# CERALIVE/ceracoder

Hardware: AMD Instinct MI355X
Metric: 1080p H.264 encoded frames/sec per GPU (higher is better)
Workload: dtype u8

## Files before the change

### ceracoder_amd/csrc/enc_handle.cpp

```cpp
#include "enc_internal.hpp"

std::atomic<int> g_open_encoders{0};
bool exclusive_device(const mi355enc_t *h) { static const bool env = getenv("MI355ENC_EXCLUSIVE") != nullptr; return h->cfg.exclusive_device != 0 || env; }
bool pgate_on(int nmb) {
    if (getenv("MI355ENC_NO_PGATE")) return false;
    const char *m = getenv("MI355ENC_PGATE_MAX");
    return nmb <= (m ? atoi(m) : 16384);
}
bool fip_on(int nmb) { return getenv("MI355ENC_NO_FIP") ? false : getenv("MI355ENC_FIP") ? true : nmb <= 3600; }
bool overlap_allowed(const mi355enc_t *h) {
    static const bool serial = getenv("MI355ENC_SERIAL") != nullptr;
    return !serial && h->safe_level == 0 && !h->cfg.single_stream && g_open_encoders.load(std::memory_order_relaxed) == 1;
}

int sync_compute(mi355enc_t *h) {
    if (h->ustream) HIPCHK(hipStreamSynchronize(h->ustream));
    HIPCHK(hipStreamSynchronize(h->fstream));
    HIPCHK(hipStreamSynchronize(h->stream));
    HIPCHK(hipStreamSynchronize(h->cstream));
    HIPCHK(hipStreamSynchronize(h->istream));
    return 0;
}

#include <mutex>
#include <vector>
static std::mutex g_pin_mu;
static std::vector<std::pair<uintptr_t, size_t>> g_pins;
bool host_range_pinned(const void *p, size_t bytes) {
    const uintptr_t a = (uintptr_t)p;
    std::lock_guard<std::mutex> g(g_pin_mu);
    for (const auto &r : g_pins)
        if (a >= r.first && a + bytes <= r.first + r.second) return true;
    return false;
}

extern "C" {

void *mi355enc_host_alloc(size_t bytes) {
    void *p = nullptr;
    if (!bytes || hipHostMalloc(&p, bytes, hipHostMallocPortable) != hipSuccess || !p) { (void)hipGetLastError(); return nullptr; }
    std::lock_guard<std::mutex> g(g_pin_mu);
    g_pins.emplace_back((uintptr_t)p, bytes);
    return p;
}
void mi355enc_host_free(void *p) {
    if (!p) return;
    {
        std::lock_guard<std::mutex> g(g_pin_mu);
        for (size_t i = 0; i < g_pins.size(); i++)
            if (g_pins[i].first == (uintptr_t)p) { g_pins.erase(g_pins.begin() + (long)i); break; }
    }
    (void)hipHostFree(p);
}

int mi355enc_abi_version(void) { return MI355ENC_ABI_VERSION; }

const char *mi355enc_strerror(int code) {
    switch (code) {
    case MI355ENC_OK: return "ok";
    case MI355ENC_ERR_ARG: return "invalid argument";
    case MI355ENC_ERR_NO_DEVICE: return "no usable HIP device (this encoder has no CPU fallback)";
    case MI355ENC_ERR_HIP: return "HIP runtime error";
    case MI355ENC_ERR_NOMEM: return "out of memory";
    case MI355ENC_ERR_OVERFLOW: return "output buffer too small";
    case MI355ENC_ERR_STATE: return "call order violated";
    default: return "unknown error";
    }
}

void mi355enc_default_cfg(mi355enc_cfg_t *c, int width, int height, int fps_num, int fps_den) {
    memset(c, 0, sizeof *c);
    c->width = width; c->height = height; c->fps_num = fps_num; c->fps_den = fps_den > 0 ? fps_den : 1;
    c->gop = 60; c->me_range = 16; c->bitrate_bps = 2048000; c->device_id = 0; c->fixed_qp = -1;
    c->qp_min = 10; c->qp_max = 51; c->pipeline_depth = 0; c->profile_events = 0; c->use_graphs = 1; c->keep_prefilter = 0; c->deblock_mode = 0; c->subpel = 1; c->i4x4 = 1; c->transform8x8 = 0; c->intra_in_p = 1; c->vbv_ms = 600; c->cavlc_threads = 0; c->intra_mode = 0; c->scenecut = 1; c->exclusive_device = 0; c->aq_mode = 0; c->single_stream = 0; c->intra_slices = 0; c->partitions = 0; c->profile_overlap = 0; c->i8x8 = 0; c->slices = 0; c->slice_deblock = 1;
}

int mi355enc_open(const mi355enc_cfg_t *cfg, mi355enc_t **out) {
    if (!cfg || !out) return MI355ENC_ERR_ARG;
    *out = nullptr;
    const double t_open = now_ms();
    if (cfg->width < 16 || cfg->height < 16 || cfg->width > 8192 || cfg->height > 8192 || (cfg->width & 1) || (cfg->height & 1) ||
        cfg->fps_num <= 0 || cfg->fps_den <= 0 || cfg->gop < 1 || cfg->me_range < 1 || cfg->me_range > 16 ||
        cfg->pipeline_depth < 0 || cfg->pipeline_depth > NSLOT - 1 || cfg->fixed_qp > 51 || cfg->slices < 0 || cfg->intra_slices < 0) {
        fprintf(stderr, "mi355enc: invalid configuration\n");
        return MI355ENC_ERR_ARG;
    }
    int ndev = 0;
    hipError_t e = hipGetDeviceCount(&ndev);
    if (e != hipSuccess || ndev <= 0 || cfg->device_id < 0 || cfg->device_id >= ndev) {
        fprintf(stderr, "mi355enc: no usable HIP device (count=%d, device-id=%d, %s); this encoder has no CPU path\n", ndev,
                cfg->device_id, e == hipSuccess ? "ok" : hipGetErrorString(e));
        return MI355ENC_ERR_NO_DEVICE;
    }
    HIPCHK(hipSetDevice(cfg->device_id));
    mi355enc_t *h = new (std::nothrow) mi355enc();
    if (!h) return MI355ENC_ERR_NOMEM;
    memset((void *)&h->cfg, 0, sizeof h->cfg);
    h->cfg = *cfg;
    if (h->cfg.qp_min <= 0 && h->cfg.qp_max <= 0) { h->cfg.qp_min = 10; h->cfg.qp_max = 51; }
    if (h->cfg.qp_max > 51) h->cfg.qp_max = 51;
    if (h->cfg.qp_min < 0) h->cfg.qp_min = 0;
    h->mbw = (cfg->width + 15) / 16; h->mbh = (cfg->height + 15) / 16;
    {
        const bool local = h->cfg.slice_deblock != 0;
        auto rows_for = [&](int n) { if (n <= 1) return 0; int rows = (h->mbh + n - 1) / n; if (local) rows = (rows + MI355_BAND_ROWS - 1) / MI355_BAND_ROWS * MI355_BAND_ROWS; return rows >= h->mbh ? 0 : rows; };
        static_assert(MI355_BAND_ROWS == 4, "the oracle rounds slice heights to multiples of four rows (orc_slice_rows_for)");
        const int nauto = h->mbh / 17 < 1 ? 1 : h->mbh / 17 > 8 ? 8 : h->mbh / 17;
        const int ns = h->cfg.intra_slices > 0 ? h->cfg.intra_slices : nauto, np = h->cfg.slices > 0 ? h->cfg.slices : nauto;
        h->islice_rows = rows_for(ns > h->mbh ? h->mbh : ns);
        h->pslice_rows = rows_for(np > h->mbh ? h->mbh : np);
        h->slice_dbf = local ? 2 : 0;
        h->stage_slice_rows = 0; h->stage_slice_dbf = 0;
    }
    h->W = h->mbw * 16; h->H = h->mbh * 16; h->nmb = h->mbw * h->mbh;
    h->ysz = (size_t)h->W * h->H; h->csz = h->ysz / 2;
    h->head = h->tail = h->pending = 0;
    h->cur = 0; h->have_ref = 0; h->frames_since_idr = 0; h->idr_count = 0; h->last_collected_rec = 0; h->last_slot = nullptr;
    h->ir_on = 0; h->ir_pos = 0; h->ir_R = 0; h->ir_skip_owed = 0;
    h->in_w = cfg->width; h->in_h = cfg->height; h->sar_w = h->sar_h = 0; h->scaling = false; h->d_scale_tab = nullptr; h->scale_tab_bytes = 0; memset(&h->scale, 0, sizeof h->scale);
    h->col_full = 0; h->col_prim = h->col_trc = h->col_mat = 2; h->in_col_set = false; csc_resolve(h);
    h->ov_len = 0; h->ov_last_have = 0; h->ov_last_len = 0; mi355enc_overlay_default_style(&h->ov_style);
    for (int l = 0; l < MI355ENC_IMAGE_LAYERS; l++) { h->img_cur[l] = nullptr; h->img_x[l] = h->img_y[l] = 0; h->img_op[l] = 256; h->img_serial[l] = 0; }
    h->img_bufs = nullptr; h->img_dev_bytes = 0; memset(h->img_last, 0, sizeof h->img_last);
    snapshot_init(h);
    h->q_on = false; h->q_have = false; h->d_qacc = nullptr; h->h_qres = nullptr; for (int i = 0; i < NSLOT; i++) h->ev_q[i] = nullptr; memset(&h->q_last, 0, sizeof h->q_last); memset(&h->q_tot, 0, sizeof h->q_tot);
    for (int i = 0; i < NSET; i++) { h->g_intra[i] = h->g_deblock[i] = nullptr; h->d_ctx2[i] = nullptr; h->d_surf[i] = nullptr; h->d_idec2[i] = nullptr; h->d_mbi_set[i] = nullptr; h->d_levels_set[i] = nullptr; h->d_qp_off[i] = nullptr; }
    h->prev_slot = nullptr;
    h->d_ctx = nullptr; h->d_pre_y = h->d_pre_uv = nullptr; memset(h->d_imv, 0, sizeof h->d_imv); h->d_psrc[0] = h->d_psrc[1] = nullptr; h->psrc_cur = 0; h->fstream = nullptr; h->ustream = nullptr; h->d_ip_strips = nullptr; h->epoch = 0; h->istream = nullptr; h->ev_pmb = nullptr; h->d_db_gran = nullptr; h->d_db_par = nullptr; h->d_ib_gran = nullptr; h->ev_dbI[0] = h->ev_dbI[1] = nullptr; h->dbI_busy[0] = h->dbI_busy[1] = 0; h->d_off = nullptr; h->d_isad = nullptr; h->d_dbrec = nullptr; h->d_idec = nullptr;
    h->cstream = nullptr; h->d_mbi = nullptr; h->d_levels = nullptr;
    memset(&h->st, 0, sizeof h->st);
    h->want_bps.store(cfg->bitrate_bps ? cfg->bitrate_bps : 2048000);
    h->fixed_qp.store(cfg->fixed_qp);
    h->fixed_drop.store(0);
    *out = h;
    g_open_encoders.fetch_add(1, std::memory_order_relaxed);
    HIPCHK(hipStreamCreateWithFlags(&h->stream, hipStreamNonBlocking));
    h->fip_rows = fip_on(h->nmb);
    h->pgate = pgate_on(h->nmb);
    {
        const int wgs_max = 256 - 256 / 4;
        for (int idr = 0; idr < 2; idr++) h->wait_room[idr] = wait_room_wgs(h->mbw, h->mbh, idr != 0, h->fip_rows) <= wgs_max;
    }
    for (int i = 0; i < NSET; i++) HIPCHK(hipMalloc((void **)&h->d_ctx2[i], sizeof(frame_ctx_t)));
    h->d_ctx = h->d_ctx2[0];
    if (h->cfg.single_stream) {
        h->cstream = h->fstream = h->istream = h->stream;
        HIPCHK(hipEventCreateWithFlags(&h->ev_pmb, hipEventDisableTiming));
    } else {
        int lo = 0, hi = 0;
        HIPCHK(hipDeviceGetStreamPriorityRange(&lo, &hi));
        HIPCHK(hipStreamCreateWithPriority(&h->cstream, hipStreamNonBlocking, hi));
        const char *rs = getenv("MI355ENC_RESERVE_CUS");
        const int nres = rs ? atoi(rs) : 0, rmode = (rs && strchr(rs, ',')) ? atoi(strchr(rs, ',') + 1) : 0;
        if (nres > 0 && nres < 200) {
            hipDeviceProp_t pr;
            HIPCHK(hipGetDeviceProperties(&pr, h->cfg.device_id));
            const int ncu = pr.multiProcessorCount;
            uint32_t mask[16];
            memset(mask, 0, sizeof mask);
            for (int i = 0; i < ncu && i < 512; i++) mask[i >> 5] |= 1u << (i & 31);
            for (int k = 0; k < nres; k++) { const int i = rmode == 1 ? (int)((long long)k * ncu / nres) : k; mask[i >> 5] &= ~(1u << (i & 31)); }
            HIPCHK(hipExtStreamCreateWithCUMask(&h->fstream, (uint32_t)((ncu + 31) / 32), mask));
            HIPCHK(hipExtStreamCreateWithCUMask(&h->istream, (uint32_t)((ncu + 31) / 32), mask));
        } else {
        HIPCHK(hipStreamCreateWithPriority(&h->fstream, hipStreamNonBlocking, getenv("MI355ENC_FPRIO") ? atoi(getenv("MI355ENC_FPRIO")) : lo));
        HIPCHK(hipStreamCreateWithPriority(&h->istream, hipStreamNonBlocking, 0));
        }
        if (h->cfg.pipeline_depth >= 1 && !getenv("MI355ENC_NO_UPSTREAM")) HIPCHK(hipStreamCreateWithFlags(&h->ustream, hipStreamNonBlocking));
        HIPCHK(hipEventCreateWithFlags(&h->ev_pmb, hipEventDisableTiming));
    }
    for (int i = 0; i < NSET; i++) {
        HIPCHK(hipMalloc((void **)&h->d_mbi_set[i], (size_t)h->nmb * sizeof(mb_info_t)));
        HIPCHK(hipMalloc((void **)&h->d_levels_set[i], (size_t)h->nmb * MB_LEVELS * sizeof(int16_t)));
        HIPCHK(hipMemsetAsync(h->d_mbi_set[i], 0, (size_t)h->nmb * sizeof(mb_info_t), h->stream));
    }
    h->d_mbi = h->d_mbi_set[0]; h->d_levels = h->d_levels_set[0]; h->n_submitted = 0;
    h->sc_sum = 0; h->sc_cnt = 0; h->sc_prev_skip = 0; h->sc_force_at = ~0ull;
    for (int i = 0; i < 2; i++) {
        HIPCHK(hipMalloc((void **)&h->d_rec_y[i], h->ysz + SURF_PAD));
        HIPCHK(hipMalloc((void **)&h->d_rec_uv[i], h->csz + SURF_PAD));
        HIPCHK(hipMemsetAsync(h->d_rec_y[i], 0, h->ysz + SURF_PAD, h->stream));
        HIPCHK(hipMemsetAsync(h->d_rec_uv[i], 0, h->csz + SURF_PAD, h->stream));
    }
    HIPCHK(hipMalloc((void **)&h->d_isad, (size_t)h->nmb * ISAD_PER_MB * sizeof(uint16_t)));
    HIPCHK(hipMalloc((void **)&h->d_dbrec, (size_t)h->nmb * 64));
    HIPCHK(hipMalloc((void **)&h->d_idec, (size_t)h->nmb * IDEC_BYTES + 16));
    h->d_idec2[0] = h->d_idec;
    { int r = h->words.alloc(h->mbh, h->stream); if (r) return r; }
    HIPCHK(hipMalloc((void **)&h->d_db_par, k_deblock_partab_bytes(h->mbw, h->mbh)));
    HIPCHK(hipMalloc((void **)&h->d_ib_gran, (size_t)h->mbh * h->mbw * 8 * sizeof(uint2)));
    HIPCHK(hipMemsetAsync(h->d_ib_gran, 0, (size_t)h->mbh * h->mbw * 8 * sizeof(uint2), h->stream));
    for (int i = 0; i < 2; i++) HIPCHK(hipEventCreateWithFlags(&h->ev_dbI[i], hipEventDisableTiming));
    HIPCHK(hipMalloc((void **)&h->d_db_gran, k_deblock_gran_bytes(h->mbw, h->mbh)));
    HIPCHK(hipMemsetAsync(h->d_db_gran, 0, k_deblock_gran_bytes(h->mbw, h->mbh), h->stream));
    HIPCHK(hipMalloc((void **)&h->d_off, (size_t)h->nmb * sizeof(unsigned)));
    for (int k = 0; k < NSET; k++) {
        HIPCHK(hipMalloc((void **)&h->d_surf[k], (size_t)h->nmb * SURF_U16 * sizeof(uint16_t)));
        for (int i = 0; i < 3; i++) HIPCHK(hipMalloc((void **)&h->d_imv[k][i], (size_t)h->nmb * sizeof(imv_t)));
        if (k > 0) HIPCHK(hipMalloc((void **)&h->d_idec2[k], (size_t)h->nmb * IDEC_BYTES + 16));
        if (h->cfg.aq_mode) HIPCHK(hipMalloc((void **)&h->d_qp_off[k], (size_t)h->nmb + 16));
    }
    for (int k = 0; k < 2; k++) {
        HIPCHK(hipMalloc((void **)&h->d_psrc[k], h->ysz + SURF_PAD));
        HIPCHK(hipMemsetAsync(h->d_psrc[k], 0, h->ysz + SURF_PAD, h->stream));
    }
    HIPCHK(hipMalloc((void **)&h->d_ip_strips, (size_t)h->nmb * IP_STRIP_BYTES));
    HIPCHK(hipMemsetAsync(h->d_ip_strips, 0, (size_t)h->nmb * IP_STRIP_BYTES, h->stream));
    if (cfg->keep_prefilter) {
        HIPCHK(hipMalloc((void **)&h->d_pre_y, h->ysz));
        HIPCHK(hipMalloc((void **)&h->d_pre_uv, h->csz));
    }
    for (int i = 0; i < NSLOT; i++) {
        slot_t *s = &h->slot[i];
        memset(s, 0, sizeof *s);
        HIPCHK(hipHostMalloc((void **)&s->h_ctx, sizeof(frame_ctx_t), hipHostMallocDefault));
        HIPCHK(hipHostMalloc((void **)&s->h_mbi, (size_t)h->nmb * sizeof(mb_info_t), hipHostMallocDefault));
        HIPCHK(hipHostMalloc((void **)&s->h_levels, (size_t)h->nmb * PACK_BLOCKS_MAX * 32, hipHostMallocDefault));
        HIPCHK(hipHostMalloc((void **)&s->h_hdr, (size_t)(4 + h->mbh) * sizeof(unsigned), hipHostMallocDefault));
        s->h_hdr[0] = s->h_hdr[1] = 0;
        HIPCHK(hipMalloc((void **)&s->d_src_y, h->ysz + SURF_PAD));
        HIPCHK(hipMalloc((void **)&s->d_src_uv, h->csz + SURF_PAD));
        HIPCHK(hipEventCreateWithFlags(&s->done, hipEventDisableTiming));
        HIPCHK(hipEventCreateWithFlags(&s->gpu_done, hipEventDisableTiming));
        HIPCHK(hipEventCreateWithFlags(&s->ev_front, hipEventDisableTiming));
        HIPCHK(hipEventCreateWithFlags(&s->ev_up, hipEventDisableTiming));
        for (int k = 0; k < 12; k++) HIPCHK(hipEventCreate(&s->ev[k]));
    }
    h->writer = h264_writer_new(h->mbw, h->mbh, h->cfg.transform8x8);
    if (!h->writer) return MI355ENC_ERR_NOMEM;
    h264_writer_set_slice_rows(h->writer, h->islice_rows);
    h264_writer_set_p_slices(h->writer, h->pslice_rows, h->slice_dbf);
    if (h->cfg.cavlc_threads <= 0) {
        const unsigned hw = std::thread::hardware_concurrency();
        int n = (int)(hw / 4);
        h->cfg.cavlc_threads = h->nmb < 1000 ? 1 : n < 1 ? 1 : n > 8 ? 8 : n;
    }
    if (h->cfg.cavlc_threads > 1 && h264_writer_set_threads(h->writer, h->cfg.cavlc_threads)) return MI355ENC_ERR_NOMEM;
    rc_init(&h->rc, (double)cfg->fps_num / cfg->fps_den, cfg->gop, h->want_bps.load(), h->cfg.qp_min, h->cfg.qp_max);
    if (h->cfg.vbv_ms > 0) rc_set_vbv(&h->rc, h->cfg.vbv_ms);
    HIPCHK(hipStreamSynchronize(h->stream));
    h->ms_open = now_ms() - t_open; h->n_skip_pictures = 0;
    h->safe_level = 0; h->n_recoveries = 0; h->last_error_word = 0;
    h->wk_qh = h->wk_qt = 0; h->wk_stop = false; h->wk_on = false; h->au_cap = 0;
    if (h->cfg.pipeline_depth >= 1 && !getenv("MI355ENC_SYNC_ENTROPY")) {
        h->au_cap = h264_max_au_bytes(h->mbw, h->mbh);
        for (int i = 0; i < NSLOT; i++) { h->slot[i].au = (uint8_t *)malloc(h->au_cap); if (!h->slot[i].au) return MI355ENC_ERR_NOMEM; }
        h->wk_on = true;
        h->wk = std::thread(entropy_worker, h);
    }
    h->stg_n = h->stg_next = h->stg_done = h->stg_err = 0; h->stg_gen = 0; h->stg_stop = false; h->stg_on = false;
    if (h->cfg.pipeline_depth >= 1 && !getenv("MI355ENC_NO_STAGE_THREADS")) {
        h->stg_on = true;
        for (auto &t : h->stg_th) t = std::thread(stage_helper, h);
    }
    return MI355ENC_OK;
}

void mi355enc_close(mi355enc_t *h) {
    if (!h) return;
    if (h->wk_on) {
        { std::lock_guard<std::mutex> g(h->wk_mu); h->wk_stop = true; }
        h->wk_cv.notify_all();
        h->wk.join();
        h->wk_on = false;
    }
    if (h->stg_on) {
        { std::lock_guard<std::mutex> g(h->stg_mu); h->stg_stop = true; }
        h->stg_cv.notify_all();
        for (auto &t : h->stg_th) t.join();
        h->stg_on = false;
    }
    g_open_encoders.fetch_sub(1, std::memory_order_relaxed);
    (void)hipSetDevice(h->cfg.device_id);
    if (h->ustream) { (void)hipStreamSynchronize(h->ustream); (void)hipStreamDestroy(h->ustream); }
    if (h->fstream) (void)hipStreamSynchronize(h->fstream);
    if (h->stream) (void)hipStreamSynchronize(h->stream);
    if (h->istream) (void)hipStreamSynchronize(h->istream);
    if (h->ev_pmb) (void)hipEventDestroy(h->ev_pmb);
    for (int i = 0; i < NSET; i++) { if (h->g_intra[i]) (void)hipGraphExecDestroy(h->g_intra[i]); if (h->g_deblock[i]) (void)hipGraphExecDestroy(h->g_deblock[i]); }
    for (int i = 0; i < NSLOT; i++) {
        slot_t *s = &h->slot[i];
        if (s->h_ctx) (void)hipHostFree(s->h_ctx);
        if (s->h_mbi) (void)hipHostFree(s->h_mbi);
        if (s->h_levels) (void)hipHostFree(s->h_levels);
        if (s->h_hdr) (void)hipHostFree(s->h_hdr);
        if (s->h_src) (void)hipHostFree(s->h_src);
        free(s->au);
        if (s->d_src_y) (void)hipFree(s->d_src_y);
        if (s->d_src_uv) (void)hipFree(s->d_src_uv);
        if (s->d_raw) (void)hipFree(s->d_raw);
        if (s->d_csc) (void)hipFree(s->d_csc);
        orient_free(s);
        jpeg_free(s);
        if (s->done) (void)hipEventDestroy(s->done);
        if (s->gpu_done) (void)hipEventDestroy(s->gpu_done);
        if (s->ev_front) (void)hipEventDestroy(s->ev_front);
        if (s->ev_up) (void)hipEventDestroy(s->ev_up);
        for (int k = 0; k < 12; k++) if (s->ev[k]) (void)hipEventDestroy(s->ev[k]);
    }
    for (int i = 0; i < 2; i++) { if (h->d_rec_y[i]) (void)hipFree(h->d_rec_y[i]); if (h->d_rec_uv[i]) (void)hipFree(h->d_rec_uv[i]); }
    if (h->d_pre_y) (void)hipFree(h->d_pre_y);
    if (h->d_pre_uv) (void)hipFree(h->d_pre_uv);
    if (h->d_isad) (void)hipFree(h->d_isad);
    if (h->d_dbrec) (void)hipFree(h->d_dbrec);
    if (h->d_idec) (void)hipFree(h->d_idec);
    h->words.release();
    if (h->d_db_gran) (void)hipFree(h->d_db_gran);
    if (h->d_db_par) (void)hipFree(h->d_db_par);
    if (h->d_ib_gran) (void)hipFree(h->d_ib_gran);
    for (int i = 0; i < 2; i++) if (h->ev_dbI[i]) (void)hipEventDestroy(h->ev_dbI[i]);
    if (h->d_off) (void)hipFree(h->d_off);
    scale_free(h);
    quality_free(h);
    snapshot_free(h);
    image_free(h);
    rate_free(h);
    hdr_free(h);
    adjust_free(h);
    autolevel_free(h);
    dspatial_free(h);
    lut3d_close(h);
    roi_free(h);
    mask_free(h);
    denoise_free(h);
    stab_free(h);
    warp_close(h);
    for (int k = 0; k < NSET; k++) {
        if (h->d_surf[k]) (void)hipFree(h->d_surf[k]);
        for (int i = 0; i < 3; i++) if (h->d_imv[k][i]) (void)hipFree(h->d_imv[k][i]);
        if (k > 0 && h->d_idec2[k]) (void)hipFree(h->d_idec2[k]);
        if (h->d_qp_off[k]) (void)hipFree(h->d_qp_off[k]);
    }
    for (int k = 0; k < 2; k++) if (h->d_psrc[k]) (void)hipFree(h->d_psrc[k]);
    if (h->d_ip_strips) (void)hipFree(h->d_ip_strips);
    for (int i = 0; i < NSET; i++) if (h->d_ctx2[i]) (void)hipFree(h->d_ctx2[i]);
    for (int i = 0; i < NSET; i++) { if (h->d_mbi_set[i]) (void)hipFree(h->d_mbi_set[i]); if (h->d_levels_set[i]) (void)hipFree(h->d_levels_set[i]); }
    if (h->cstream && h->cstream != h->stream) { (void)hipStreamSynchronize(h->cstream); (void)hipStreamDestroy(h->cstream); }
    if (h->fstream && h->fstream != h->stream) (void)hipStreamDestroy(h->fstream);
    if (h->istream && h->istream != h->stream) (void)hipStreamDestroy(h->istream);
    if (h->stream) (void)hipStreamDestroy(h->stream);
    h264_writer_free(h->writer);
    delete h;
}

int mi355enc_set_bitrate(mi355enc_t *h, uint32_t bps) {
    if (!h) return MI355ENC_ERR_ARG;
    h->want_bps.store(bps < 1000 ? 1000 : bps, std::memory_order_relaxed);
    return MI355ENC_OK;
}
uint32_t mi355enc_get_bitrate(const mi355enc_t *h) { return h ? h->want_bps.load(std::memory_order_relaxed) : 0; }
int mi355enc_set_fixed_qp(mi355enc_t *h, int qp) {
    if (!h || qp > 51) return MI355ENC_ERR_ARG;
    h->fixed_qp.store(qp < 0 ? -1 : qp, std::memory_order_relaxed);
    return MI355ENC_OK;
}
int mi355enc_set_fixed_drop(mi355enc_t *h, int drop) {
    if (!h || drop < 0 || (drop > DROP_MAX && drop != DROP_SKIP)) return MI355ENC_ERR_ARG;
    h->fixed_drop.store(drop, std::memory_order_relaxed);
    return MI355ENC_OK;
}
int mi355enc_set_intra_refresh(mi355enc_t *h, int on) {
    if (!h || h->n_submitted) return MI355ENC_ERR_ARG;
    if (on && (h->cfg.intra_in_p == 0 || h->cfg.partitions || h->cfg.gop < 2 || h->cfg.gop > MI355ENC_IR_MAX_PERIOD)) return MI355ENC_ERR_ARG;
    h->ir_on = on ? 1 : 0;
    return MI355ENC_OK;
}
int mi355enc_pending(const mi355enc_t *h) { return h ? h->pending : 0; }
size_t mi355enc_max_au_bytes(const mi355enc_t *h) { return h ? h264_max_au_bytes(h->mbw, h->mbh) : 0; }
int mi355enc_mb_width(const mi355enc_t *h) { return h ? h->mbw : 0; }
int mi355enc_mb_height(const mi355enc_t *h) { return h ? h->mbh : 0; }

int mi355enc_get_stats(mi355enc_t *h, mi355enc_stats_t *st) {
    if (!h || !st) return MI355ENC_ERR_ARG;
    *st = h->st;
    st->target_bps = h->want_bps.load();
    st->cavlc_threads = (uint32_t)h->cfg.cavlc_threads;
    st->ms_open = h->ms_open; st->skip_pictures = h->n_skip_pictures;
    st->recoveries = h->n_recoveries; st->last_error_word = h->last_error_word; st->safe_level = (uint32_t)h->safe_level;
    return MI355ENC_OK;
}
void mi355enc_reset_stats(mi355enc_t *h) { if (h) { memset(&h->st, 0, sizeof h->st); h->n_skip_pictures = 0; memset(&h->q_tot, 0, sizeof h->q_tot); } }

int mi355enc_fetch(mi355enc_t *h, int what, void *dst, size_t n) {
    if (!h || !dst) return MI355ENC_ERR_ARG;
    HIPCHK(hipSetDevice(h->cfg.device_id));
    const void *src = nullptr; size_t need = 0; bool host = false;
    switch (what) {
    case MI355ENC_FETCH_RECON_Y: src = h->d_rec_y[h->last_collected_rec]; need = h->ysz; break;
    case MI355ENC_FETCH_RECON_UV: src = h->d_rec_uv[h->last_collected_rec]; need = h->csz; break;
    case MI355ENC_FETCH_PREFILTER_Y: src = h->d_pre_y; need = h->ysz; break;
    case MI355ENC_FETCH_PREFILTER_UV: src = h->d_pre_uv; need = h->csz; break;
    case MI355ENC_FETCH_MBINFO: src = h->last_slot ? h->last_slot->h_mbi : nullptr; need = (size_t)h->nmb * sizeof(mb_info_t); host = true; break;
    case MI355ENC_FETCH_SOURCE_Y: src = h->last_slot && h->last_slot->src_y == h->last_slot->d_src_y ? h->last_slot->d_src_y : nullptr; need = h->ysz; break;
    case MI355ENC_FETCH_SOURCE_UV: src = h->last_slot && h->last_slot->src_y == h->last_slot->d_src_y ? h->last_slot->d_src_uv : nullptr; need = h->csz; break;
    case MI355ENC_FETCH_SCALE_TABLES: src = h->d_scale_tab; need = h->scale_tab_bytes; break;
    case MI355ENC_FETCH_LEVELS: src = h->last_slot ? h->d_levels_set[h->last_slot->set] : nullptr; need = (size_t)h->nmb * MB_LEVELS * 2; break;
    case 102: case 103: case 104: {
        if (!h->words.fetch_bytes(what)) return MI355ENC_ERR_STATE;
        if (n < h->words.fetch_bytes(what)) return MI355ENC_ERR_OVERFLOW;
        int r = sync_compute(h);
        return r ? r : h->words.fetch(what, dst);
    }
    case 100: src = h->d_dbrec; need = (size_t)h->nmb * 64; break;
    case 101: src = h->d_isad; need = 1024; break;
    default: return MI355ENC_ERR_ARG;
    }
    if (!src) return MI355ENC_ERR_STATE;
    if (n < need) return MI355ENC_ERR_OVERFLOW;
    if (host) { memcpy(dst, src, need); return MI355ENC_OK; }
    { int r = sync_compute(h); if (r) return r; }
    HIPCHK(hipMemcpy(dst, src, need, hipMemcpyDeviceToHost));
    return MI355ENC_OK;
}

}
```

### ceracoder_amd/csrc/k_motion.hip

```cpp
#include "kernels_common.hpp"

#ifndef ME_MBS
#define ME_MBS 4
#endif
#define ME_WQ (ME_MBS + 2)
#define ME_ROWS 50
#define ME_STRIDE 53
#define ME_K 5

DEV unsigned long long qsad(unsigned lo, unsigned hi, unsigned cur, unsigned long long acc) {
    unsigned long long src = ((unsigned long long)hi << 32) | lo;
    return __builtin_amdgcn_qsad_pk_u16_u8(src, cur, acc);
}
DEV int mv_bits(int v) {
    int a = iabs(v);
    return a == 0 ? 1 : 7 + 2 * (31 - __clz(a));
}
DEV int med3(int a, int b, int c) {
    const int lo = a < b ? a : b, hi = a < b ? b : a;
    return c < lo ? lo : (c > hi ? hi : c);
}
struct fpred_t { int px, py, sx, sy; };
DEV fpred_t field_pred(const imv_t *__restrict__ f, int mbw, int mx, int my, bool top) {
    const bool avA = mx > 0, avB = top, avC = top && mx + 1 < mbw, avD = mx > 0 && top, hasC = avC || avD;
    const int self = my * mbw + mx;
    const unsigned wa = avA ? ldg32(f + self - 1) : 0u, wb = avB ? ldg32(f + self - mbw) : 0u;
    const unsigned wc = avC ? ldg32(f + self - mbw + 1) : (avD ? ldg32(f + self - mbw - 1) : 0u);
    const int ax = (int)(int16_t)(wa & 0xFFFF), ay = (int)(int16_t)(wa >> 16), bx = (int)(int16_t)(wb & 0xFFFF), by = (int)(int16_t)(wb >> 16);
    const int cx = (int)(int16_t)(wc & 0xFFFF), cy = (int)(int16_t)(wc >> 16);
    const int n = (avA ? 1 : 0) + (avB ? 1 : 0) + (hasC ? 1 : 0);
    fpred_t r;
    if (n == 1) { r.px = avA ? ax : avB ? bx : cx; r.py = avA ? ay : avB ? by : cy; }
    else { r.px = med3(ax, bx, cx); r.py = med3(ay, by, cy); }
    const bool zero = !avA || !avB || wa == 0u || wb == 0u;
    r.sx = zero ? 0 : r.px; r.sy = zero ? 0 : r.py;
    return r;
}
template <bool ZERO = false>
DEV unsigned select_min(const unsigned long long *acc, int g, int dxg, bool active, int R, int lambda, int px, int py, int sx, int sy) {
    const unsigned INVALID = 0x40000000u;
    unsigned bo[4];
#pragma unroll
    for (int o = 0; o < 4; o++) {
        const int dx = -16 + 4 * dxg + o;
        bo[o] = (dx >= -R && dx <= R && active) ? (((unsigned)(lambda * mv_bits(dx - px)) << 12) | (unsigned)(dx + 16)) : INVALID;
    }
    const int so = sx + 16 - 4 * dxg;
    unsigned best = 0xFFFFFFFFu;
#pragma unroll
    for (int d = 0; d < ME_K; d++) {
        const int dy = -16 + ME_K * g + d;
        const unsigned pos = (unsigned)(dy + 16) << 6;
        const unsigned bd = (dy >= -R && dy <= R) ? (((unsigned)(lambda * (mv_bits(dy - py) + SEL_BONUS)) << 12) | pos) : INVALID;
        const unsigned lo = (unsigned)acc[d], hi = (unsigned)(acc[d] >> 32);
        unsigned s[4] = {(lo << 16) >> 4, (lo & 0xFFFF0000u) >> 4, (hi << 16) >> 4, (hi & 0xFFFF0000u) >> 4};
        unsigned k[4];
#pragma unroll
        for (int o = 0; o < 4; o++) {
            const bool is_skip = !ZERO && dy == sy && so == o && active;
            k[o] = is_skip ? (s[o] | pos | (unsigned)(sx + 16)) : s[o] + bd + bo[o];
        }
        unsigned ka = k[0] < k[1] ? k[0] : k[1], kb = k[2] < k[3] ? k[2] : k[3];
        ka = ka < kb ? ka : kb;
        best = best < ka ? best : ka;
    }
    if (ZERO && active && ME_K * g <= 16 && 16 < ME_K * g + ME_K && dxg == 4) {
        const unsigned long long a = acc[16 - ME_K * (16 / ME_K)];
        const unsigned k0 = (((unsigned)a << 16) >> 4) | (16u << 6) | 16u;
        best = best < k0 ? best : k0;
    }
    return wave64_umin(best);
}
DEV void store_imv(imv_t *dst, unsigned best, int lambda, int px, int py, int sx, int sy) {
    const int bx = (int)(best & 63) - 16, by = (int)((best >> 6) & 63) - 16;
    const unsigned bits = (bx == sx && by == sy) ? 0u : (unsigned)(mv_bits(bx - px) + mv_bits(by - py) + SEL_BONUS);
    const unsigned sad = (best >> 12) - (unsigned)lambda * bits;
    stg64(dst, make_uint2(((unsigned)(uint16_t)(4 * bx)) | ((unsigned)(uint16_t)(4 * by) << 16), sad | (bits << 16)));
}

__global__ __launch_bounds__(64 * ME_MBS) void me_kernel(const frame_ctx_t cv, int row0) {
    const frame_ctx_t *__restrict__ ctx = &cv;
    if (blockIdx.x == 0) tl_first(ctx, 0);
    __shared__ unsigned win[ME_ROWS * ME_STRIDE];
    const int stride = ctx->stride, mbw = ctx->mbw, mbh = ctx->mbh;
    const int W = mbw * 16, H = mbh * 16;
    const int strips = (mbw + ME_MBS - 1) / ME_MBS;
    const int tile = xcd_remap(blockIdx.x, gridDim.x);
    const int my = row0 + tile / strips, sx = tile % strips;
    const int t = threadIdx.x;
    const uint8_t *__restrict__ ref = ctx->me_ref_y;

    for (int i = t; i < 48 * ME_WQ; i += 64 * ME_MBS) {
        int row = i / ME_WQ, q = i - row * ME_WQ;
        const int gy = clip3(0, H - 1, my * 16 - 16 + row), gx = sx * (ME_MBS * 16) - 16 + 16 * q;
        uint4 v;
#ifdef ME_DBG_NOSTAGE
        v = make_uint4(i, i, i, i);
        if (gx != -12345) {}
#else
        if (gx >= 0 && gx < W) v = ldg128(ref + (size_t)gy * stride + gx);
#endif
        else { const unsigned e = ldg8(ref + (size_t)gy * stride + (gx < 0 ? 0 : W - 1)) * 0x01010101u; v = make_uint4(e, e, e, e); }
        unsigned *d = &win[row * ME_STRIDE + 4 * q];
        d[0] = v.x; d[1] = v.y; d[2] = v.z; d[3] = v.w;
    }
    if (t < ME_ROWS) win[t * ME_STRIDE + 4 * ME_WQ] = 0;
    if (t < 2 * (4 * ME_WQ + 1)) win[(48 + t / (4 * ME_WQ + 1)) * ME_STRIDE + t % (4 * ME_WQ + 1)] = 0;

    const int lane = t & 63, m = t >> 6;
    const int mx = sx * ME_MBS + m;
    const bool active = lane < 63 && mx < mbw;
    const int g = lane < 63 ? lane / 9 : 0, dxg = lane < 63 ? lane % 9 : 0;
    const int mxc = mx < mbw ? mx : mbw - 1;

    unsigned c[16][4];
    {
        const uint8_t *__restrict__ src = ctx->src_y;
        const int ss = ctx->src_stride, vh = ctx->vis_h;
        const int mu = __builtin_amdgcn_readfirstlane(mxc);
#pragma unroll
        for (int r = 0; r < 16; r++) {
            int sy = my * 16 + r;
            sy = sy < vh ? sy : vh - 1;
#ifdef ME_DBG_NOCUR
            const uint4 v = make_uint4(sy, mu, r, sy ^ mu);
#else
            const uint4 v = ldc128(src + (size_t)sy * ss + mu * 16);
#endif
            c[r][0] = __builtin_amdgcn_readfirstlane(v.x); c[r][1] = __builtin_amdgcn_readfirstlane(v.y);
            c[r][2] = __builtin_amdgcn_readfirstlane(v.z); c[r][3] = __builtin_amdgcn_readfirstlane(v.w);
        }
        if (lane < 16 && mx < mbw) {
            int sy = my * 16 + lane;
            sy = sy < vh ? sy : vh - 1;
            stg128(ctx->psrc_out + (size_t)(my * 16 + lane) * stride + mu * 16, ldg128(src + (size_t)sy * ss + mu * 16));
        }
    }
    __syncthreads();

    unsigned long long acc[ME_K];
#pragma unroll
    for (int d = 0; d < ME_K; d++) acc[d] = 0;
    const unsigned *wp = &win[(ME_K * g) * ME_STRIDE + 4 * m + dxg];
#ifdef ME_DBG_REPEAT
    for (int rep = 0; rep < ME_DBG_REPEAT; rep++) {
#endif
    unsigned w0 = wp[0], w1 = wp[1], w2 = wp[2], w3 = wp[3], w4 = wp[4];
#pragma unroll
    for (int j = 0; j < 16 + ME_K - 1; j++) {
        unsigned n0 = 0, n1 = 0, n2 = 0, n3 = 0, n4 = 0;
        if (j + 1 < 16 + ME_K - 1) {
            n0 = wp[(j + 1) * ME_STRIDE + 0]; n1 = wp[(j + 1) * ME_STRIDE + 1]; n2 = wp[(j + 1) * ME_STRIDE + 2];
            n3 = wp[(j + 1) * ME_STRIDE + 3]; n4 = wp[(j + 1) * ME_STRIDE + 4];
        }
#pragma unroll
        for (int d = 0; d < ME_K; d++) {
            const int r = j - d;
            if (r >= 0 && r < 16) {
                acc[d] = qsad(w0, w1, c[r][0], acc[d]);
                acc[d] = qsad(w1, w2, c[r][1], acc[d]);
                acc[d] = qsad(w2, w3, c[r][2], acc[d]);
                acc[d] = qsad(w3, w4, c[r][3], acc[d]);
            }
        }
        asm volatile("" : "+v"(acc[0]), "+v"(acc[1]), "+v"(acc[2]), "+v"(acc[3]), "+v"(acc[4]));
        __builtin_amdgcn_sched_barrier(0);
        w0 = n0; w1 = n1; w2 = n2; w3 = n3; w4 = n4;
    }
#ifdef ME_DBG_REPEAT
    }
#endif
#ifdef ME_DBG_NOSURF
    if (active && acc[0] == 0x123456789ull) {
#else
    if (active) {
#endif
        uint16_t *sf = ctx->surf + (size_t)(my * mbw + mx) * SURF_U16 + 4 * dxg;
#pragma unroll
        for (int d = 0; d < ME_K; d++) stg64(sf + (ME_K * g + d) * SURF_COLS, make_uint2((unsigned)acc[d], (unsigned)(acc[d] >> 32)));
    }
#ifdef ME_DBG_NOSEL
    const unsigned best = ((((unsigned)acc[0] ^ (unsigned)acc[4]) & 0x0FFFu) << 12) | 0x410u;
#else
    const unsigned best = select_min<true>(acc, g, dxg, active, ctx->me_range, ctx->lambda, 0, 0, 0, 0);
#endif
    if (lane == 0 && mx < mbw) store_imv(&ctx->imv_a[my * mbw + mx], best, ctx->lambda, 0, 0, 0, 0);
    tl_last(ctx, 1);
}

__global__ __launch_bounds__(256) void me_select_kernel(const frame_ctx_t cv, int mb0, int mb1, const imv_t *__restrict__ in, imv_t *__restrict__ out,
                                                        const imv_t *__restrict__ prev, int mode) {
    const frame_ctx_t *__restrict__ ctx = &cv;
    const int mbw = ctx->mbw;
    const int lane = threadIdx.x & 63, wave = __builtin_amdgcn_readfirstlane(threadIdx.x >> 6);
    const int mbn = mb0 + xcd_remap(blockIdx.x, gridDim.x) * 4 + wave;
    if (mbn >= mb1) return;
    const int my = mbn / mbw, mx = mbn - my * mbw;
    const fpred_t fp = field_pred(in, mbw, mx, my, row_has_top(ctx, my));
    const int px = fp.px >> 2, py = fp.py >> 2, sx = fp.sx >> 2, sy = fp.sy >> 2;
    if (mode) {
        fpred_t fq = {0, 0, 0, 0};
        if (mode == 2) fq = field_pred(prev, mbw, mx, my, row_has_top(ctx, my));
        if (px == (fq.px >> 2) && py == (fq.py >> 2) && sx == (fq.sx >> 2) && sy == (fq.sy >> 2)) {
            if (lane == 0) stg64(&out[mbn], ldg64(&in[mbn]));
            return;
        }
    }
    const bool active = lane < 63;
    const int g = active ? lane / 9 : 0, dxg = active ? lane % 9 : 0;
    unsigned long long acc[ME_K];
    const uint16_t *sf = ctx->surf + (size_t)mbn * SURF_U16 + 4 * dxg;
#pragma unroll
    for (int d = 0; d < ME_K; d++) { const uint2 v = ldg64(sf + (ME_K * g + d) * SURF_COLS); acc[d] = ((unsigned long long)v.y << 32) | v.x; }
    const unsigned best = select_min(acc, g, dxg, active, ctx->me_range, ctx->lambda, px, py, sx, sy);
    if (lane == 0) store_imv(&out[mbn], best, ctx->lambda, px, py, sx, sy);
}

#ifndef SEL_SPW
#define SEL_SPW 8
#endif
__global__ __launch_bounds__(256) void me_select_sparse_kernel(const frame_ctx_t cv, int mb0, int mb1, const imv_t *__restrict__ in, imv_t *__restrict__ out, const imv_t *__restrict__ prev) {
    const frame_ctx_t *__restrict__ ctx = &cv;
    const int mbw = ctx->mbw;
    const int lane = threadIdx.x & 63, wave = __builtin_amdgcn_readfirstlane(threadIdx.x >> 6);
    const int base = mb0 + ((int)blockIdx.x * 4 + wave) * SEL_SPW;
    if (base >= mb1) return;
    const int mine = base + (lane < SEL_SPW ? lane : 0);
    const bool have = lane < SEL_SPW && mine < mb1;
    const int mbn_l = have ? mine : base, my_l = mbn_l / mbw, mx_l = mbn_l - my_l * mbw;
    const bool top_l = row_has_top(ctx, my_l);
    const fpred_t fp = field_pred(in, mbw, mx_l, my_l, top_l), fq = field_pred(prev, mbw, mx_l, my_l, top_l);
    const int px = fp.px >> 2, py = fp.py >> 2, sx = fp.sx >> 2, sy = fp.sy >> 2;
    const bool same = px == (fq.px >> 2) && py == (fq.py >> 2) && sx == (fq.sx >> 2) && sy == (fq.sy >> 2);
    if (have && same) stg64(&out[mbn_l], ldg64(&in[mbn_l]));
    unsigned todo = (unsigned)(__ballot(have && !same) & ((1ull << SEL_SPW) - 1ull));
    const bool active = lane < 63;
    const int g = active ? lane / 9 : 0, dxg = active ? lane % 9 : 0;
    while (todo) {
        const int j = __builtin_ctz(todo);
        todo &= todo - 1;
        const int mbn = base + j;
        const int jpx = __builtin_amdgcn_readlane(px, j), jpy = __builtin_amdgcn_readlane(py, j), jsx = __builtin_amdgcn_readlane(sx, j), jsy = __builtin_amdgcn_readlane(sy, j);
        unsigned long long acc[ME_K];
        const uint16_t *sf = ctx->surf + (size_t)mbn * SURF_U16 + 4 * dxg;
#pragma unroll
        for (int d = 0; d < ME_K; d++) { const uint2 v = ldg64(sf + (ME_K * g + d) * SURF_COLS); acc[d] = ((unsigned long long)v.y << 32) | v.x; }
        const unsigned best = select_min(acc, g, dxg, active, ctx->me_range, ctx->lambda, jpx, jpy, jsx, jsy);
        if (lane == 0) store_imv(&out[mbn], best, ctx->lambda, jpx, jpy, jsx, jsy);
    }
}

#define SP_GS 24
#define SP_PS 20
struct sp_lds {
    uint8_t G[23 * SP_GS];
    int16_t H1[18 * SP_GS];
    uint8_t b[19 * SP_PS];
    uint8_t h[18 * SP_GS];
    uint8_t j[18 * SP_PS];
    uint8_t pad[16];
};
typedef short sp_s2 __attribute__((ext_vector_type(2)));
DEV sp_s2 as_s2(unsigned v) { return __builtin_bit_cast(sp_s2, v); }
DEV unsigned as_u(sp_s2 v) { return __builtin_bit_cast(unsigned, v); }
DEV sp_s2 bytes_lo(unsigned w) { return as_s2(__builtin_amdgcn_perm(0u, w, 0x0c010c00u)); }
DEV sp_s2 bytes_hi(unsigned w) { return as_s2(__builtin_amdgcn_perm(0u, w, 0x0c030c02u)); }
DEV sp_s2 clip255_s2(sp_s2 v) { return __builtin_elementwise_min(__builtin_elementwise_max(v, (sp_s2)(0)), (sp_s2)(255)); }
DEV sp_s2 pair_s2(int a, int b) { return as_s2(__builtin_amdgcn_perm((unsigned)b, (unsigned)a, 0x05040100u)); }
DEV unsigned pack_s2(sp_s2 lo, sp_s2 hi) { return __builtin_amdgcn_perm(as_u(hi), as_u(lo), 0x06040200u); }
DEV unsigned clip_pack4(int a, int b, int c, int d) { return pack_s2(clip255_s2(pair_s2(a, b)), clip255_s2(pair_s2(c, d))); }
DEV int mvq_bits(int q) {
    unsigned k = q > 0 ? (unsigned)(2 * q - 1) : (unsigned)(-2 * q);
    return 2 * (31 - __clz((int)(k + 1))) + 1;
}
DEV unsigned lds4(const uint8_t *plane, int o) {
    const unsigned *w = (const unsigned *)(plane + (o & ~3));
    return __builtin_amdgcn_alignbyte(w[1], w[0], (unsigned)(o & 3));
}
DEV unsigned sp_sample4(const sp_lds *L, int X, int Y, int fx, int fy) {
#define SG(x, y) lds4(L->G, ((y) + 2) * SP_GS + (x) + 2)
#define SB(x, y) lds4(L->b, (y) * SP_PS + (x))
#define SH(x, y) lds4(L->h, (y) * SP_GS + (x) + 2)
#define SJ(x, y) lds4(L->j, (y) * SP_PS + (x))
    if (fy == 0) {
        if (fx == 0) return SG(X, Y);
        return fx == 2 ? SB(X, Y) : fx == 1 ? avg4(SG(X, Y), SB(X, Y)) : avg4(SG(X + 1, Y), SB(X, Y));
    }
    if (fx == 0) return fy == 2 ? SH(X, Y) : fy == 1 ? avg4(SG(X, Y), SH(X, Y)) : avg4(SG(X, Y + 1), SH(X, Y));
    if ((fx & 1) && (fy & 1)) return avg4(fy == 1 ? SB(X, Y) : SB(X, Y + 1), fx == 1 ? SH(X, Y) : SH(X + 1, Y));
    if (fx == 2 && fy == 2) return SJ(X, Y);
    if (fx == 2) return avg4(fy == 1 ? SB(X, Y) : SB(X, Y + 1), SJ(X, Y));
    return avg4(fx == 1 ? SH(X, Y) : SH(X + 1, Y), SJ(X, Y));
#undef SG
#undef SB
#undef SH
#undef SJ
}
DEV void sp_planes(sp_lds *L, const int lane) {
    if (lane < 54) {
        const int d = lane % 6, seg = lane / 6;
        sp_s2 lo[7], hi[7];
#pragma unroll
        for (int r = 0; r < 7; r++) {
            const unsigned w = *(const unsigned *)&L->G[(2 * seg + r) * SP_GS + 4 * d];
            lo[r] = bytes_lo(w); hi[r] = bytes_hi(w);
        }
#pragma unroll
        for (int t = 0; t < 2; t++) {
            const sp_s2 vl = (lo[t + 2] + lo[t + 3]) * (sp_s2)(20) - (lo[t + 1] + lo[t + 4]) * (sp_s2)(5) + (lo[t] + lo[t + 5]);
            const sp_s2 vh = (hi[t + 2] + hi[t + 3]) * (sp_s2)(20) - (hi[t + 1] + hi[t + 4]) * (sp_s2)(5) + (hi[t] + hi[t + 5]);
            const int R = 2 * seg + t;
            unsigned *o = (unsigned *)&L->H1[R * SP_GS + 4 * d];
            o[0] = as_u(vl); o[1] = as_u(vh);
            *(unsigned *)&L->h[R * SP_GS + 4 * d] = pack_s2(clip255_s2((vl + (sp_s2)(16)) >> (sp_s2)(5)), clip255_s2((vh + (sp_s2)(16)) >> (sp_s2)(5)));
        }
    }
#pragma unroll
    for (int it = 0; it < 2; it++) {
        const int i = lane + 64 * it;
        if (i < 19 * 5) {
            const int R = i / 5, g = i - R * 5;
            const unsigned *gw = (const unsigned *)&L->G[(R + 2) * SP_GS + 4 * g];
            const unsigned d0 = gw[0] ^ 0x80808080u, d1 = gw[1] ^ 0x80808080u, d2 = gw[2] ^ 0x80808080u;
            int o[4];
#pragma unroll
            for (int k = 0; k < 4; k++) {
                const unsigned w0 = k ? __builtin_amdgcn_alignbyte(d1, d0, (unsigned)k) : d0, w1 = k ? __builtin_amdgcn_alignbyte(d2, d1, (unsigned)k) : d1;
                const int v = __builtin_amdgcn_sdot4((int)w0, 0x1414FB01, __builtin_amdgcn_sdot4((int)w1, 0x000001FB, 4096, false), false);
                o[k] = (v + 16) >> 5;
            }
            *(unsigned *)&L->b[R * SP_PS + 4 * g] = clip_pack4(o[0], o[1], o[2], o[3]);
        }
    }
    WAVE_SYNC();
#pragma unroll
    for (int it = 0; it < 2; it++) {
        const int i = lane + 64 * it;
        if (i < 18 * 5) {
            const int R = i / 5, g = i - R * 5;
            const unsigned *hw = (const unsigned *)&L->H1[R * SP_GS + 4 * g];
            const unsigned p0 = hw[0], p1 = hw[1], p2 = hw[2], p3 = hw[3], p4 = hw[4];
            const unsigned q0 = __builtin_amdgcn_alignbyte(p1, p0, 2u), q1 = __builtin_amdgcn_alignbyte(p2, p1, 2u),
                           q2 = __builtin_amdgcn_alignbyte(p3, p2, 2u), q3 = __builtin_amdgcn_alignbyte(p4, p3, 2u);
            const sp_s2 ca = {1, -5}, cb = {20, 20}, cc = {-5, 1};
#define J3(a, b, c) __builtin_amdgcn_sdot2(as_s2(a), ca, __builtin_amdgcn_sdot2(as_s2(b), cb, __builtin_amdgcn_sdot2(as_s2(c), cc, 512, false), false), false)
            const int v0 = J3(p0, p1, p2), v1 = J3(q0, q1, q2), v2 = J3(p1, p2, p3), v3 = J3(q1, q2, q3);
#undef J3
            *(unsigned *)&L->j[R * SP_PS + 4 * g] = clip_pack4(v0 >> 10, v1 >> 10, v2 >> 10, v3 >> 10);
        }
    }
    WAVE_SYNC();
}
__global__ __launch_bounds__(256) void subpel_kernel(const frame_ctx_t cv, int mb0, int mb1) {
    const frame_ctx_t *__restrict__ ctx = &cv;
    __shared__ __attribute__((aligned(16))) sp_lds LD[4];
    const int mbw = ctx->mbw, mbh = ctx->mbh, stride = ctx->stride, W = mbw * 16, H = mbh * 16;
    const int lane = threadIdx.x & 63, wave = __builtin_amdgcn_readfirstlane(threadIdx.x >> 6);
    int mbn = mb0 + blockIdx.x * 4 + wave;
    const bool ok = mbn < mb1;
    if (!ok) mbn = mb1 - 1;
    const int my = mbn / mbw, mx = mbn - my * mbw, x0 = mx * 16, y0 = my * 16;
    sp_lds *L = &LD[wave];
    const mb_info_t info = ld_mbinfo(&ctx->mbi[mbn]);
    const int ix = x0 + (info.mvx >> 2), iy = y0 + (info.mvy >> 2);
    const uint8_t *__restrict__ ref = ctx->ref_y;
    if (ix - 3 >= 0 && iy - 3 >= 0 && ((ix - 3) & ~3) + 28 <= W && iy + 19 < H) {
        const int a = (ix - 3) & 3;
        const uint8_t *base = ref + (size_t)(iy - 3) * stride + ((ix - 3) & ~3);
        for (int i = lane; i < 23 * 6; i += 64) {
            const int r = i / 6, d = i - r * 6;
            const unsigned w0 = ldg32(base + (size_t)r * stride + 4 * d), w1 = ldg32(base + (size_t)r * stride + 4 * d + 4);
            *(unsigned *)&L->G[r * SP_GS + 4 * d] = __builtin_amdgcn_alignbyte(w1, w0, (unsigned)a);
        }
    } else
        for (int i = lane; i < 23 * 23; i += 64) {
            int r = i / 23, c = i - r * 23;
            int yy = clip3(0, H - 1, iy - 3 + r), xx = clip3(0, W - 1, ix - 3 + c);
            L->G[r * SP_GS + c] = (uint8_t)ldg8(ref + (size_t)yy * stride + xx);
        }
    const int pr = lane >> 2, pc = (lane & 3) * 4;
    unsigned curw;
    {
        int sy = y0 + pr;
        sy = sy < ctx->vis_h ? sy : ctx->vis_h - 1;
        curw = ldg32(ctx->src_y + (size_t)sy * ctx->src_stride + x0 + pc);
    }
    WAVE_SYNC();
    sp_planes(L, lane);
    const int lambda = ctx->lambda;
    int bqx = info.mvx, bqy = info.mvy;
    unsigned best = info.cost;
#pragma unroll 1
    for (int step = 2; step >= 1; step--) {
        const int cqx = bqx, cqy = bqy;
        unsigned acc[4] = {0, 0, 0, 0};
#pragma unroll
        for (int c8 = 0; c8 < 8; c8++) {
            const int k = c8 < 4 ? c8 : c8 + 1;
            const int qx = cqx + (k % 3 - 1) * step, qy = cqy + (k / 3 - 1) * step;
            const int ox = qx - info.mvx, oy = qy - info.mvy;
            const int X = 1 + (ox >> 2) + pc, Y = 1 + (oy >> 2) + pr;
            const unsigned sad = __builtin_amdgcn_sad_u8(curw, sp_sample4(L, X, Y, ox & 3, oy & 3), 0u);
            acc[c8 >> 1] |= sad << (16 * (c8 & 1));
        }
#pragma unroll
        for (int q = 0; q < 4; q++) {
            acc[q] = (unsigned)wave64_sum((int)acc[q]);
        }
#pragma unroll
        for (int c8 = 0; c8 < 8; c8++) {
            const int k = c8 < 4 ? c8 : c8 + 1;
            const int qx = cqx + (k % 3 - 1) * step, qy = cqy + (k / 3 - 1) * step;
            const unsigned sad = (acc[c8 >> 1] >> (16 * (c8 & 1))) & 0xFFFFu;
            const unsigned cost = sad + (unsigned)(lambda * (mvq_bits(qx) + mvq_bits(qy)));
            if (cost < best) { best = cost; bqx = qx; bqy = qy; }
        }
    }
    if (lane == 0 && ok) {
        mb_info_t *mb = &ctx->mbi[mbn];
        stg32(&mb->mvx, ((unsigned)(uint16_t)bqx) | ((unsigned)(uint16_t)bqy << 16));
        stg32(&mb->cost, best);
    }
}

DEV int dec_score(unsigned M) { return dec_score_mask(M); }
DEV int row_or4(int v) {
    v |= __builtin_amdgcn_update_dpp(0, v, 0x128, 0xF, 0xF, false);
    v |= __builtin_amdgcn_update_dpp(0, v, 0x124, 0xF, 0xF, false);
    return v;
}
DEV unsigned ref_word4(const uint8_t *__restrict__ ref, int stride, int W, int H, int x, int y, bool inside) {
    if (inside) {
        const uint8_t *b = ref + (size_t)y * stride + (x & ~3);
        return __builtin_amdgcn_alignbyte(ldg32(b + 4), ldg32(b), (unsigned)(x & 3));
    }
    const uint8_t *r = ref + (size_t)clip3(0, H - 1, y) * stride;
    return pack4((int)ldg8(r + clip3(0, W - 1, x)), (int)ldg8(r + clip3(0, W - 1, x + 1)), (int)ldg8(r + clip3(0, W - 1, x + 2)), (int)ldg8(r + clip3(0, W - 1, x + 3)));
}
DEV void chroma_pred4(const frame_ctx_t *__restrict__ ctx, int lane, int x0, int y0, int W, int H, int mvx, int mvy, int *pd) {
    const int stride = ctx->stride;
    const int py = (lane >> 2) & 3, cby = (lane >> 4) & 1, c = (lane >> 1) & 1, cbx = lane & 1;
    const int cx0 = x0 >> 1, cy0 = y0 >> 1, cw = W >> 1, ch = H >> 1;
    const int cy = cby * 4 + py, cxb = cbx * 4;
    const int xi = mvx >> 3, yi = mvy >> 3, xf = mvx & 7, yf = mvy & 7;
    const uint8_t *__restrict__ rf = ctx->ref_uv;
    int A[5], B[5];
    if (cx0 + xi >= 0 && cx0 + xi + 9 <= cw && cy0 + yi >= 0 && cy0 + yi + 9 <= ch) {
        const int o = 2 * (cx0 + cxb + xi) + c, a = o & 3;
        const uint8_t *r0 = rf + (size_t)(cy0 + cy + yi) * stride + (o & ~3), *r1 = r0 + stride;
        const unsigned a0 = ldg32(r0), a1 = ldg32(r0 + 4), a2 = ldg32(r0 + 8), b0 = ldg32(r1), b1 = ldg32(r1 + 4), b2 = ldg32(r1 + 8);
        const unsigned sa0 = __builtin_amdgcn_alignbyte(a1, a0, (unsigned)a), sa1 = __builtin_amdgcn_alignbyte(a2, a1, (unsigned)a);
        const unsigned sb0 = __builtin_amdgcn_alignbyte(b1, b0, (unsigned)a), sb1 = __builtin_amdgcn_alignbyte(b2, b1, (unsigned)a);
        A[0] = byte_of(sa0, 0); A[1] = byte_of(sa0, 2); A[2] = byte_of(sa1, 0); A[3] = byte_of(sa1, 2); A[4] = (int)((a2 >> (8 * a)) & 255);
        B[0] = byte_of(sb0, 0); B[1] = byte_of(sb0, 2); B[2] = byte_of(sb1, 0); B[3] = byte_of(sb1, 2); B[4] = (int)((b2 >> (8 * a)) & 255);
    } else {
        const int ya = clip3(0, ch - 1, cy0 + cy + yi), yb = clip3(0, ch - 1, cy0 + cy + yi + 1);
#pragma unroll
        for (int i = 0; i < 5; i++) {
            const int xx = clip3(0, cw - 1, cx0 + cxb + i + xi);
            A[i] = (int)ldg8(rf + (size_t)ya * stride + 2 * xx + c);
            B[i] = (int)ldg8(rf + (size_t)yb * stride + 2 * xx + c);
        }
    }
    const int w00 = (8 - xf) * (8 - yf), w10 = xf * (8 - yf), w01 = (8 - xf) * yf, w11 = xf * yf;
#pragma unroll
    for (int i = 0; i < 4; i++) pd[i] = (w00 * A[i] + w10 * A[i + 1] + w01 * B[i] + w11 * B[i + 1] + 32) >> 6;
}
DEV unsigned pmb_luma_tq(const dev_tables *T, int lane, unsigned curw, unsigned pw, int qp, bool decimate, int *lev, int *x) {
    const int py = (lane >> 2) & 3, fy = ((py & 1) << 1) | (py >> 1);
    const col_bf cb = make_col_bf(py);
    const int kz0 = (int)((0xFEA9DB83C7426510ull >> (16 * fy)) & 0xFFFF);
    const qparams q = make_q(T, qp, false);
    const int mfe = py < 2 ? q.mf[0] : q.mf[2], mfo = py < 2 ? q.mf[2] : q.mf[1], ve = py < 2 ? q.v[0] : q.v[2], vo = py < 2 ? q.v[2] : q.v[1];
#pragma unroll
    for (int i = 0; i < 4; i++) x[i] = byte_of(curw, i) - byte_of(pw, i);
    fwd_rows4(x);
    unsigned m = 0, big = 0;
#pragma unroll
    for (int i = 0; i < 4; i++) {
        const int cf = fwd_col(x[i], cb);
        lev[i] = quant1(cf, (i & 1) ? mfo : mfe, q.f, q.qbits);
        m |= (lev[i] != 0 ? 1u : 0u) << ((kz0 >> (4 * i)) & 15);
        big |= (lev[i] > 1 || lev[i] < -1) ? 1u : 0u;
    }
    if (decimate) {
        const unsigned mm = (unsigned)row_or4((int)(m | (big << 16)));
        int s = (mm >> 16) ? 9 : dec_score(((mm & 0xFFFFu) << 1) | 1u);
        int s8 = s + quad_xor<1>(s);
        s8 += __shfl_xor(s8, 16, 64);
        int tot = s8 + quad_xor<2>(s8);
        tot += __shfl_xor(tot, 32, 64);
        if (s8 < 4 || tot < 6) { lev[0] = lev[1] = lev[2] = lev[3] = 0; }
    }
#pragma unroll
    for (int i = 0; i < 4; i++) x[i] = (lev[i] * ((i & 1) ? vo : ve)) << q.shift;
    const unsigned long long bal = __ballot((lev[0] | lev[1] | lev[2] | lev[3]) != 0);
    const unsigned long long t = bal | (bal >> 4) | (bal >> 8) | (bal >> 12);
    const int rb = lane & 15, rbx = blkx(rb) >> 2, rby = blky(rb) >> 2;
    return (unsigned)(__ballot(lane < 16 && ((t >> (16 * rby + rbx)) & 1)) & 0xFFFFull);
}
DEV unsigned pmb_satd(int lane, unsigned curw, unsigned pw) {
    const int py = (lane >> 2) & 3, s1 = py < 2 ? 1 : -1, s2 = (py & 1) ? -1 : 1;
    const int d0 = byte_of(curw, 0) - byte_of(pw, 0), d1 = byte_of(curw, 1) - byte_of(pw, 1), d2 = byte_of(curw, 2) - byte_of(pw, 2), d3 = byte_of(curw, 3) - byte_of(pw, 3);
    const int a = d0 + d3, b = d1 + d2, c = d1 - d2, e = d0 - d3;
    int t[4] = {a + b, e + c, a - b, e - c};
    int acc = 0;
#pragma unroll
    for (int i = 0; i < 4; i++) {
        const int u = mad24(t[i], s1, row_xor8(t[i]));
        const int w = mad24(u, s2, row_xor4(u));
        acc += iabs(w);
    }
    return (unsigned)wave64_sum(acc);
}
DEV unsigned pmb_sa8d(int lane, unsigned curw, unsigned pw) {
    const int s0 = (lane & 1) ? -1 : 1, s1 = (lane & 4) ? -1 : 1, s2 = (lane & 8) ? -1 : 1, s3 = (lane & 16) ? -1 : 1;
    const int d0 = byte_of(curw, 0) - byte_of(pw, 0), d1 = byte_of(curw, 1) - byte_of(pw, 1), d2 = byte_of(curw, 2) - byte_of(pw, 2), d3 = byte_of(curw, 3) - byte_of(pw, 3);
    const int a = d0 + d3, b = d1 + d2, c = d1 - d2, e = d0 - d3;
    int t[4] = {a + b, e + c, a - b, e - c};
    int acc = 0;
#pragma unroll
    for (int i = 0; i < 4; i++) {
        int u = mad24(t[i], s0, quad_xor<1>(t[i]));
        u = mad24(u, s1, row_xor4(u));
        u = mad24(u, s2, row_xor8(u));
        u = mad24(u, s3, __shfl_xor(u, 16, 64));
        acc += iabs(u);
    }
    return (unsigned)wave64_sum(acc);
}
DEV bool pmb_pick_t8(int lane, unsigned curw, unsigned pw) {
    const unsigned raw4 = pmb_satd(lane, curw, pw), raw8 = pmb_sa8d(lane, curw, pw);
    return __builtin_amdgcn_readfirstlane((int)(((raw8 + 2) >> 2) < (raw4 >> 1))) != 0;
}
template <bool SC1>
DEV void pmb_store_pred_only(const frame_ctx_t *__restrict__ ctx, int16_t *lv, int lane, int x0, int y0, unsigned pw, const int *pd) {
    const int stride = ctx->stride, pr = lane >> 2, pc = (lane & 3) * 4;
    stx32<SC1>(ctx->rec_y + (size_t)(y0 + pr) * stride + x0 + pc, pw);
    const int py = (lane >> 2) & 3, cby = (lane >> 4) & 1, c = (lane >> 1) & 1, cbx = lane & 1;
    const unsigned mine = pack4(pd[0], pd[1], pd[2], pd[3]), other = (unsigned)quad_xor<2>((int)mine);
    if (lane < 32 && c == 0) {
        uint2 out;
        out.x = __builtin_amdgcn_perm(other, mine, 0x05010400u);
        out.y = __builtin_amdgcn_perm(other, mine, 0x07030602u);
        stx64<SC1>(ctx->rec_uv + (size_t)((y0 >> 1) + cby * 4 + py) * stride + 2 * ((x0 >> 1) + cbx * 4), out);
    }
    if (lane < MB_LEVELS * 2 / 16) stg128(lv + 8 * lane, make_uint4(0, 0, 0, 0));
}

template <bool SC1>
DEV unsigned pmb_luma_t8(const frame_ctx_t *__restrict__ ctx, int *tile, int lane, unsigned curw, unsigned pw, int qp, int mbn, int x0, int y0) {
    const int pr = lane >> 2, pc = (lane & 3) * 4;
    {
        int *t = tile + ((pr >> 3) * 2 + (pc >> 3)) * 64 + (pr & 7) * 8 + (pc & 7);
#pragma unroll
        for (int i = 0; i < 4; i++) t[i] = byte_of(curw, i) - byte_of(pw, i);
    }
    WAVE_SYNC();
    const bool act = lane < 16;
    const int i8 = (lane >> 2) & 3, j = lane & 3;
    int *tb = tile + i8 * 64;
    const int m6 = qp % 6, k6 = qp / 6;
    int rs[2][8], cw[2][8];
    unsigned submask = 0;
    if (act) {
#pragma unroll
        for (int r = 0; r < 2; r++) {
#pragma unroll
            for (int i = 0; i < 8; i++) rs[r][i] = tb[(2 * j + r) * 8 + i];
            fdct8_1d(rs[r]);
        }
    }
    WAVE_SYNC();
    if (act) {
#pragma unroll
        for (int r = 0; r < 2; r++)
#pragma unroll
            for (int i = 0; i < 8; i++) tb[(2 * j + r) * 8 + i] = rs[r][i];
    }
    WAVE_SYNC();
    if (act) {
#pragma unroll
        for (int c2 = 0; c2 < 2; c2++) {
#pragma unroll
            for (int r = 0; r < 8; r++) cw[c2][r] = tb[r * 8 + 2 * j + c2];
            fdct8_1d(cw[c2]);
#pragma unroll
            for (int r = 0; r < 8; r++) {
                const int xx = 2 * j + c2, cl = pos_class8(r, xx);
                const int qbits = 16 + k6, f = (1 << qbits) / 6;
                const int a = iabs(cw[c2][r]);
                int l = (int)(((long long)a * g_tab.mf8[m6][cl] + f) >> qbits);
                l = l > 2047 ? 2047 : l;
                l = cw[c2][r] < 0 ? -l : l;
                const int kk = g_tab.izz8[r * 8 + xx];
                stg16(&ctx->levels[(size_t)mbn * MB_LEVELS + L_LUMA + (4 * i8 + (kk & 3)) * 16 + (kk >> 2)], l);
                if (l) submask |= 1u << (kk & 3);
                const int ls = 16 * g_tab.v8[m6][cl];
                cw[c2][r] = qp >= 36 ? (l * ls) << (k6 - 6) : (l * ls + (1 << (5 - k6))) >> (6 - k6);
            }
        }
    }
    WAVE_SYNC();
    if (act) {
#pragma unroll
        for (int c2 = 0; c2 < 2; c2++)
#pragma unroll
            for (int r = 0; r < 8; r++) tb[r * 8 + 2 * j + c2] = cw[c2][r];
    }
    submask |= (unsigned)quad_xor<1>((int)submask);
    submask |= (unsigned)quad_xor<2>((int)submask);
    WAVE_SYNC();
    if (act) {
#pragma unroll
        for (int r = 0; r < 2; r++) {
#pragma unroll
            for (int i = 0; i < 8; i++) rs[r][i] = tb[(2 * j + r) * 8 + i];
            idct8_1d(rs[r]);
        }
    }
    WAVE_SYNC();
    if (act) {
#pragma unroll
        for (int r = 0; r < 2; r++)
#pragma unroll
            for (int i = 0; i < 8; i++) tb[(2 * j + r) * 8 + i] = rs[r][i];
    }
    WAVE_SYNC();
    if (act) {
#pragma unroll
        for (int c2 = 0; c2 < 2; c2++) {
#pragma unroll
            for (int r = 0; r < 8; r++) cw[c2][r] = tb[r * 8 + 2 * j + c2];
            idct8_1d(cw[c2]);
        }
    }
    WAVE_SYNC();
    if (act) {
#pragma unroll
        for (int c2 = 0; c2 < 2; c2++)
#pragma unroll
            for (int r = 0; r < 8; r++) tb[r * 8 + 2 * j + c2] = (cw[c2][r] + 32) >> 6;
    }
    WAVE_SYNC();
    {
        const int *t = tile + ((pr >> 3) * 2 + (pc >> 3)) * 64 + (pr & 7) * 8 + (pc & 7);
        int o[4];
#pragma unroll
        for (int i = 0; i < 4; i++) o[i] = clip255(byte_of(pw, i) + t[i]);
        stx32<SC1>(ctx->rec_y + (size_t)(y0 + pr) * ctx->stride + x0 + pc, pack4(o[0], o[1], o[2], o[3]));
    }
    return (unsigned)(__ballot(act && ((submask >> j) & 1u)) & 0xFFFFull);
}
DEV unsigned part_gsum(unsigned v) {
    v += (unsigned)quad_xor<1>((int)v);
    v += (unsigned)row_xor4((int)v);
    v += (unsigned)row_xor8((int)v);
    v += (unsigned)__shfl_xor((int)v, 16, 64);
    return v;
}
DEV unsigned part_total(unsigned g) { g += (unsigned)quad_xor<2>((int)g); return g + (unsigned)__shfl_xor((int)g, 32, 64); }
#ifdef PMB_PROF
#define PMB_NPH 11
#define PMB_MARK(k) do { const unsigned long long t1_ = __builtin_readcyclecounter(); ph_[k] = t1_ - t0_; t0_ = t1_; } while (0)
#define PMB_MARK0() unsigned long long ph_[PMB_NPH] = {0, 0, 0, 0, 0, 0, 0, 0, 0, 0, 0}; unsigned long long t0_ = __builtin_readcyclecounter()
#define PMB_FLUSH() do { if (lane == 0) for (int k_ = 0; k_ < PMB_NPH; k_++) stg32((unsigned *)ctx->dbrec + (size_t)mbn * 16 + k_, (unsigned)ph_[k_]); } while (0)
#else
#define PMB_MARK(k) ((void)0)
#define PMB_MARK0() ((void)0)
#define PMB_FLUSH() ((void)0)
#endif
struct pmb_pre_t { uint2 selfw; fpred_t fp; unsigned curw; uint2 sw; unsigned ds; uint4 dw; };
DEV pmb_pre_t pmb_preload(const frame_ctx_t *__restrict__ ctx, const int mbn, const int lane) {
    const int mbw = ctx->mbw, my = mbn / mbw, mx = mbn - my * mbw, x0 = mx * 16, y0 = my * 16;
    pmb_pre_t p;
    const imv_t *__restrict__ field = k_final_imv_dev(ctx);
    p.selfw = ldg64(field + mbn);
    {
        int sy = y0 + (lane >> 2);
        sy = sy < ctx->vis_h ? sy : ctx->vis_h - 1;
        p.curw = ldg32(ctx->src_y + (size_t)sy * ctx->src_stride + x0 + (lane & 3) * 4);
    }
    {
        const int cby = (lane >> 4) & 1, cbx = lane & 1;
        int sy = (y0 >> 1) + cby * 4 + ((lane >> 2) & 3);
        const int vh2 = ctx->vis_h >> 1;
        sy = sy < vh2 ? sy : vh2 - 1;
        p.sw = ldg64(ctx->src_uv + (size_t)sy * ctx->src_stride + 2 * ((x0 >> 1) + cbx * 4));
    }
    p.dw = ctx->intra_p ? ldg128(ctx->idec + (size_t)mbn * IDEC_BYTES + 16) : make_uint4(0, 0, 0, 0);
    p.fp = field_pred(field, mbw, mx, my, row_has_top(ctx, my));
    p.ds = (unsigned)*(const GAS uint16_t *)(ctx->surf + (size_t)mbn * SURF_U16 + ((p.fp.sy >> 2) + 16) * SURF_COLS + (p.fp.sx >> 2) + 16);
    return p;
}
DEV bool ir_ok(const frame_ctx_t *__restrict__ ctx, int mx, int mvx) {
    return mx >= ctx->ir_c0 || (16 * mx + 15 + (mvx >> 2) + ((mvx & 3) ? 3 : 0) <= ctx->ir_clean && 8 * mx + 7 + (mvx >> 3) + ((mvx & 7) ? 1 : 0) <= (ctx->ir_clean >> 1));
}
DEV int ir_max_whole(const frame_ctx_t *__restrict__ ctx, int mx) {
    const int kl = ctx->ir_clean - 16 * mx - 15, kc = 2 * ((ctx->ir_clean >> 1) - 8 * mx - 7);
    return 4 * (kl < kc ? kl : kc);
}
template <bool SC1>
DEV void pmb_store_intra(mb_info_t *mb, const uint4 dw, int qp, int lane) {
    if (lane == 0) {
        const bool i4 = ((dw.x >> 16) & 255u) != 0;
        mb_info_t m;
        m.mvx = 0; m.mvy = 0; m.mb_type = i4 ? 2 : 0; m.i16_mode = i4 ? 0 : (uint8_t)(dw.x & 255u); m.chroma_mode = (uint8_t)((dw.x >> 8) & 255u);
        m.qp = (uint8_t)qp; m.nzmask = 0; m.cost = dw.y;
        st_mbinfo_x<SC1>(mb, m);
    }
}
template <bool SC1, bool PART, int T8, bool IR>
DEV void pmb_mb(const frame_ctx_t *__restrict__ ctx, sp_lds *L, const int mbn, const int lane, const int refine, const pmb_pre_t &pre) {
    const int mbw = ctx->mbw, mbh = ctx->mbh, stride = ctx->stride, W = mbw * 16, H = mbh * 16, qp = mb_qp_dev(ctx, mbn), lambda = ctx->lambda;
    const int my = mbn / mbw, mx = mbn - my * mbw, x0 = mx * 16, y0 = my * 16;
    const dev_tables *T = &g_tab;
    PMB_MARK0();
    const uint2 selfw = pre.selfw;
    int imx = (int)(int16_t)(selfw.x & 0xFFFF);
    const int imy = (int)(int16_t)(selfw.x >> 16);
    const unsigned di = selfw.y & 0xFFFFu, ibits = selfw.y >> 16;
    const fpred_t fp = pre.fp;
    const int pr = lane >> 2, pc = (lane & 3) * 4;
    const int py = (lane >> 2) & 3;
    const unsigned curw = pre.curw;
    int sv[4];
    {
        const int c = (lane >> 1) & 1;
        const uint2 sw = pre.sw;
        const unsigned slo = c ? (sw.x >> 8) : sw.x, shi = c ? (sw.y >> 8) : sw.y;
        sv[0] = (int)(slo & 255); sv[1] = (int)((slo >> 16) & 255); sv[2] = (int)(shi & 255); sv[3] = (int)((shi >> 16) & 255);
    }
    int16_t *lv = ctx->levels + (size_t)mbn * MB_LEVELS;
    mb_info_t *mb = &ctx->mbi[mbn];
    if (IR && mx >= ctx->ir_c0 && mx < ctx->ir_c1) {
        pmb_store_intra<SC1>(mb, pre.dw, qp, lane);
        PMB_FLUSH();
        return;
    }
    {
        const unsigned ds = pre.ds;
        const bool skip_ok = !IR || ir_ok(ctx, mx, fp.sx);
        bool pass = ctx->drop_sad && ds < ctx->drop_sad && skip_ok;
        const bool worth = ds <= di + (unsigned)(lambda * SKIP_MARGIN_BITS) && skip_ok;
        PMB_MARK(0);
        if (pass || worth) {
            const int X = x0 + (fp.sx >> 2), Y = y0 + (fp.sy >> 2);
            const bool inside = X >= 0 && Y >= 0 && X + 16 <= W && Y + 16 <= H;
            const unsigned pw = ref_word4(ctx->ref_y, stride, W, H, X + pc, Y + pr, inside);
            int pd[4];
            chroma_pred4(ctx, lane, x0, y0, W, H, fp.sx, fp.sy, pd);
            if (!pass) {
                int lev[4], x[4];
                if (pmb_luma_tq(T, lane, curw, pw, qp, true, lev, x) == 0) {
                    unsigned nz_c = 0, dc_c = 0;
                    chroma_rows4(ctx, T, lv, x0 >> 1, y0 >> 1, lane, pd, sv, qp, false, false, nullptr, nz_c, dc_c, true, 0, SC1);
                    pass = (nz_c | dc_c) == 0;
                }
            }
            PMB_MARK(1);
            if (pass) {
                pmb_store_pred_only<SC1>(ctx, lv, lane, x0, y0, pw, pd);
                if (lane == 0) {
                    mb_info_t m;
                    m.mvx = (int16_t)fp.sx; m.mvy = (int16_t)fp.sy; m.mb_type = 1; m.i16_mode = 0; m.chroma_mode = 0; m.qp = (uint8_t)qp; m.nzmask = 0; m.cost = di;
                    st_mbinfo_x<SC1>(mb, m);
                }
                PMB_FLUSH();
                return;
            }
        }
    }
    if (IR && !ir_ok(ctx, mx, imx)) imx = ir_max_whole(ctx, mx);
    const int ix = x0 + (imx >> 2), iy = y0 + (imy >> 2);
    const uint8_t *__restrict__ ref = ctx->ref_y;
    if (ix - 3 >= 0 && iy - 3 >= 0 && ((ix - 3) & ~3) + 28 <= W && iy + 19 < H) {
        const int a = (ix - 3) & 3;
        const uint8_t *base = ref + (size_t)(iy - 3) * stride + ((ix - 3) & ~3);
        for (int i = lane; i < 23 * 6; i += 64) {
            const int r = i / 6, d = i - r * 6;
            const unsigned w0 = ldg32(base + (size_t)r * stride + 4 * d), w1 = ldg32(base + (size_t)r * stride + 4 * d + 4);
            *(unsigned *)&L->G[r * SP_GS + 4 * d] = __builtin_amdgcn_alignbyte(w1, w0, (unsigned)a);
        }
    } else
        for (int i = lane; i < 23 * 23; i += 64) {
            int r = i / 23, c = i - r * 23;
            int yy = clip3(0, H - 1, iy - 3 + r), xx = clip3(0, W - 1, ix - 3 + c);
            L->G[r * SP_GS + c] = (uint8_t)ldg8(ref + (size_t)yy * stride + xx);
        }
    WAVE_SYNC();
    PMB_MARK(2);
    int bqx = imx, bqy = imy;
    unsigned q0 = 0, qh[4] = {0, 0, 0, 0}, qq[4] = {0, 0, 0, 0};
    int hbx = imx, hby = imy;
    unsigned best;
    if (PART) {
        q0 = part_gsum(__builtin_amdgcn_sad_u8(curw, sp_sample4(L, 1 + pc, 1 + pr, 0, 0), 0u));
        best = part_total(q0) + (unsigned)(lambda * (mvq_bits(imx - fp.px) + mvq_bits(imy - fp.py)));
    } else
        best = (unsigned)wave64_sum((int)__builtin_amdgcn_sad_u8(curw, sp_sample4(L, 1 + pc, 1 + pr, 0, 0), 0u)) +
               (unsigned)(lambda * (mvq_bits(imx - fp.px) + mvq_bits(imy - fp.py)));
    PMB_MARK(3);
    if (refine) {
        sp_planes(L, lane);
        PMB_MARK(4);
        {
            const int cqx = bqx, cqy = bqy;
            unsigned acc[4] = {0, 0, 0, 0};
#pragma unroll
            for (int c8 = 0; c8 < 8; c8++) {
                const int k = c8 < 4 ? c8 : c8 + 1;
                const int qx = cqx + (k % 3 - 1) * 2, qy = cqy + (k / 3 - 1) * 2;
                const int ox = qx - imx, oy = qy - imy;
                const unsigned sad = __builtin_amdgcn_sad_u8(curw, sp_sample4(L, 1 + (ox >> 2) + pc, 1 + (oy >> 2) + pr, ox & 3, oy & 3), 0u);
                acc[c8 >> 1] |= sad << (16 * (c8 & 1));
            }
#pragma unroll
            for (int q = 0; q < 4; q++) {
                if (PART) { qh[q] = part_gsum(acc[q]); acc[q] = part_total(qh[q]); }
                else acc[q] = (unsigned)wave64_sum((int)acc[q]);
            }
#pragma unroll
            for (int c8 = 0; c8 < 8; c8++) {
                const int k = c8 < 4 ? c8 : c8 + 1;
                const int qx = cqx + (k % 3 - 1) * 2, qy = cqy + (k / 3 - 1) * 2;
                const unsigned sad = (acc[c8 >> 1] >> (16 * (c8 & 1))) & 0xFFFFu;
                const unsigned cost = sad + (unsigned)(lambda * (mvq_bits(qx - fp.px) + mvq_bits(qy - fp.py)));
                if (cost < best && (!IR || ir_ok(ctx, mx, qx))) { best = cost; bqx = qx; bqy = qy; }
            }
        }
        hbx = bqx; hby = bqy;
        PMB_MARK(5);
        {
            const int cqx = bqx, cqy = bqy;
            {
                const int ox = cqx - imx, oy = cqy - imy;
                best = (pmb_satd(lane, curw, sp_sample4(L, 1 + (ox >> 2) + pc, 1 + (oy >> 2) + pr, ox & 3, oy & 3)) >> 1) +
                       (unsigned)(lambda * (mvq_bits(cqx - fp.px) + mvq_bits(cqy - fp.py)));
            }
#pragma unroll 1
            for (int k = 0; k < 9; k++) {
                if (k == 4) continue;
                const int qx = cqx + (k % 3 - 1), qy = cqy + (k / 3 - 1);
                const int ox = qx - imx, oy = qy - imy;
                const unsigned cw = sp_sample4(L, 1 + (ox >> 2) + pc, 1 + (oy >> 2) + pr, ox & 3, oy & 3);
                if (PART) {
                    const int c8 = k < 4 ? k : k - 1;
                    const unsigned g = part_gsum(__builtin_amdgcn_sad_u8(curw, cw, 0u)) << (16 * (c8 & 1));
                    qq[0] |= (c8 >> 1) == 0 ? g : 0u; qq[1] |= (c8 >> 1) == 1 ? g : 0u; qq[2] |= (c8 >> 1) == 2 ? g : 0u; qq[3] |= (c8 >> 1) == 3 ? g : 0u;
                }
                const unsigned d = pmb_satd(lane, curw, cw) >> 1;
                const unsigned cost = d + (unsigned)(lambda * (mvq_bits(qx - fp.px) + mvq_bits(qy - fp.py)));
                if (cost < best && (!IR || ir_ok(ctx, mx, qx))) { best = cost; bqx = qx; bqy = qy; }
            }
        }
    }
    PMB_MARK(6);
    const int ox = bqx - imx, oy = bqy - imy;
    unsigned pw = sp_sample4(L, 1 + (ox >> 2) + pc, 1 + (oy >> 2) + pr, ox & 3, oy & 3);
    unsigned dsad = (unsigned)wave64_sum((int)__builtin_amdgcn_sad_u8(curw, pw, 0u));
    unsigned jinter = dsad + (unsigned)(lambda * (mvq_bits(bqx - fp.px) + mvq_bits(bqy - fp.py)));
    int shape = 0, lvx = bqx, lvy = bqy;
    if (PART && refine) {
        unsigned k8 = 0xFFFFFFFFu, k168 = 0xFFFFFFFFu, k816 = 0xFFFFFFFFu;
#pragma unroll 1
        for (int k = 0; k < 17; k++) {
            const int cx = k == 0 ? imx : k < 9 ? imx + (((k - 1 < 4 ? k - 1 : k) % 3) - 1) * 2 : hbx + (((k - 9 < 4 ? k - 9 : k - 8) % 3) - 1);
            const int cy = k == 0 ? imy : k < 9 ? imy + (((k - 1 < 4 ? k - 1 : k) / 3) - 1) * 2 : hby + (((k - 9 < 4 ? k - 9 : k - 8) / 3) - 1);
            const unsigned bits = (unsigned)(lambda * (mvq_bits(cx - fp.px) + mvq_bits(cy - fp.py)));
            const int c8 = k == 0 ? 0 : k < 9 ? k - 1 : k - 9;
            const unsigned pk = k == 0 ? q0 : k < 9 ? ((c8 >> 1) == 0 ? qh[0] : (c8 >> 1) == 1 ? qh[1] : (c8 >> 1) == 2 ? qh[2] : qh[3])
                                                    : ((c8 >> 1) == 0 ? qq[0] : (c8 >> 1) == 1 ? qq[1] : (c8 >> 1) == 2 ? qq[2] : qq[3]);
            const unsigned sq = k == 0 ? pk : (pk >> (16 * (c8 & 1))) & 0xFFFFu;
            const unsigned sh = sq + (unsigned)quad_xor<2>((int)sq);
            const unsigned sv_ = sq + (unsigned)__shfl_xor((int)sq, 32, 64);
            const unsigned a = ((sq + bits) << 5) | (unsigned)k, b = ((sh + bits) << 5) | (unsigned)k, c = ((sv_ + bits) << 5) | (unsigned)k;
            k8 = a < k8 ? a : k8; k168 = b < k168 ? b : k168; k816 = c < k816 ? c : k816;
        }
        const unsigned c8x8 = (k8 >> 5), c168 = (k168 >> 5), c816 = (k816 >> 5);
        unsigned t8 = c8x8 + (unsigned)quad_xor<2>((int)c8x8); t8 += (unsigned)__shfl_xor((int)t8, 32, 64);
        const unsigned t168 = c168 + (unsigned)__shfl_xor((int)c168, 32, 64);
        const unsigned t816 = c816 + (unsigned)quad_xor<2>((int)c816);
        unsigned jb = jinter + (unsigned)lambda;
        unsigned key = 0;
        const unsigned j1 = t168 + 3u * (unsigned)lambda, j2 = t816 + 3u * (unsigned)lambda, j3 = t8 + 9u * (unsigned)lambda;
        if (j1 < jb) { jb = j1; shape = 1; key = k168; }
        if (j2 < jb) { jb = j2; shape = 2; key = k816; }
        if (j3 < jb) { jb = j3; shape = 3; key = k8; }
        shape = __builtin_amdgcn_readfirstlane(shape);
        if (shape) {
            const int k = (int)(key & 31u);
            lvx = k == 0 ? imx : k < 9 ? imx + (((k - 1 < 4 ? k - 1 : k) % 3) - 1) * 2 : hbx + (((k - 9 < 4 ? k - 9 : k - 8) % 3) - 1);
            lvy = k == 0 ? imy : k < 9 ? imy + (((k - 1 < 4 ? k - 1 : k) / 3) - 1) * 2 : hby + (((k - 9 < 4 ? k - 9 : k - 8) / 3) - 1);
            const int px_ = lvx - imx, py_ = lvy - imy;
            pw = sp_sample4(L, 1 + (px_ >> 2) + pc, 1 + (py_ >> 2) + pr, px_ & 3, py_ & 3);
            dsad = (unsigned)wave64_sum((int)__builtin_amdgcn_sad_u8(curw, pw, 0u));
            jinter = jb - (unsigned)lambda;
        }
    }
    if (ctx->intra_p && di + (unsigned)lambda * ibits >= INTRA_GATE(lambda)) {
        const uint4 dw = pre.dw;
        const unsigned jintra = dw.z + (dw.z >> 3) + (unsigned)(lambda * 12);
        if (jintra < jinter) {
            pmb_store_intra<SC1>(mb, dw, qp, lane);
            PMB_FLUSH();
            return;
        }
    }
    PMB_MARK(7);
    int pd[4];
    unsigned slot = 0;
    if (PART && shape) {
        const int src = (((lane >> 4) & 1) << 5) | ((lane & 1) << 1);
        const int cvx = __shfl(lvx, src, 64), cvy = __shfl(lvy, src, 64);
        chroma_pred4(ctx, lane, x0, y0, W, H, cvx, cvy, pd);
        const unsigned mine = ((unsigned)(uint16_t)lvx) | ((unsigned)(uint16_t)lvy << 16);
        const unsigned v1 = (unsigned)__shfl((int)mine, shape == 1 ? 32 : 2, 64), v2 = (unsigned)__shfl((int)mine, 32, 64), v3 = (unsigned)__shfl((int)mine, 34, 64);
        slot = lane == 0 ? v1 : (shape == 3 && lane == 1) ? v2 : (shape == 3 && lane == 2) ? v3 : 0u;
        bqx = __builtin_amdgcn_readfirstlane(lvx); bqy = __builtin_amdgcn_readfirstlane(lvy);
    } else chroma_pred4(ctx, lane, x0, y0, W, H, bqx, bqy, pd);
    if (ctx->drop_sad && dsad < ctx->drop_sad) {
        pmb_store_pred_only<SC1>(ctx, lv, lane, x0, y0, pw, pd);
        if (PART && shape && lane < 8) stx32<SC1>(lv + L_LDC + 2 * lane, slot);
        if (lane == 0) {
            mb_info_t m;
            m.mvx = (int16_t)bqx; m.mvy = (int16_t)bqy; m.mb_type = 1; m.i16_mode = (uint8_t)shape; m.chroma_mode = 0; m.qp = (uint8_t)qp; m.nzmask = 0; m.cost = di;
            st_mbinfo_x<SC1>(mb, m);
        }
        PMB_FLUSH();
        return;
    }
    PMB_MARK(8);
    unsigned nz_luma;
    const bool t8 = T8 == 1 || (T8 == 2 && pmb_pick_t8(lane, curw, pw));
    if (t8) {
        nz_luma = pmb_luma_t8<SC1>(ctx, (int *)L, lane, curw, pw, qp, mbn, x0, y0);
    } else {
        const int fy = ((py & 1) << 1) | (py >> 1);
        const col_bf cb = make_col_bf(py);
        const int kz0 = (int)((0xFEA9DB83C7426510ull >> (16 * fy)) & 0xFFFF);
        int lev[4], x[4];
        nz_luma = pmb_luma_tq(T, lane, curw, pw, qp, true, lev, x);
        const int bx = lane & 3, by = lane >> 4, b = ((by >> 1) << 3) | ((bx >> 1) << 2) | ((by & 1) << 1) | (bx & 1);
#pragma unroll
        for (int i = 0; i < 4; i++) stg16(&lv[L_LUMA + b * 16 + ((kz0 >> (4 * i)) & 15)], lev[i]);
        inv_rows4(x);
        int o[4];
#pragma unroll
        for (int i = 0; i < 4; i++) o[i] = clip255(byte_of(pw, i) + ((inv_col(x[i], cb) + 32) >> 6));
        stx32<SC1>(ctx->rec_y + (size_t)(y0 + pr) * stride + x0 + pc, pack4(o[0], o[1], o[2], o[3]));
    }
    PMB_MARK(9);
    unsigned nz_c = 0, dc_c = 0;
    chroma_rows4(ctx, T, lv, x0 >> 1, y0 >> 1, lane, pd, sv, qp, false, true, nullptr, nz_c, dc_c, true, 0, SC1);
    PMB_MARK(10);
    if (lane == 0) {
        unsigned nzm = nz_luma | (nz_c << 16);
        if (dc_c & 1) nzm |= NZ_CBDC;
        if (dc_c & 2) nzm |= NZ_CRDC;
        if (t8 && nz_luma) nzm |= NZ_T8;
        mb_info_t m;
        m.mvx = (int16_t)bqx; m.mvy = (int16_t)bqy; m.mb_type = 1; m.i16_mode = (uint8_t)shape; m.chroma_mode = 0; m.qp = (uint8_t)qp; m.nzmask = nzm; m.cost = di;
        st_mbinfo_x<SC1>(mb, m);
    }
    if (PART && shape) { if (lane < 8) stx32<SC1>(lv + L_LDC + 2 * lane, slot); }
    else if (lane < 2) stg128(lv + L_LDC + 8 * lane, make_uint4(0, 0, 0, 0));
    PMB_FLUSH();
}

template <bool GATED, bool ROWS, bool PART, int T8, bool IR = false>
__global__ __launch_bounds__(256) void pmb_kernel(const frame_ctx_t cv, int mb0, int mb1, int refine, const unsigned *__restrict__ gate_done, unsigned ref_epoch, unsigned *err, unsigned *row_done) {
    const frame_ctx_t *__restrict__ ctx = &cv;
    __shared__ __attribute__((aligned(16))) sp_lds LD[4];
    const int lane = threadIdx.x & 63, wave = __builtin_amdgcn_readfirstlane(threadIdx.x >> 6);
    const int mbn = mb0 + 4 * (int)blockIdx.x + wave;
    if (mb0 == 0 && blockIdx.x == 0) tl_first(ctx, 2);
    pmb_pre_t pre;
    if (mbn < mb1) pre = pmb_preload(ctx, mbn, lane);
    if (GATED) {
        if (wave == 0) {
            const int mbw = ctx->mbw, mbh = ctx->mbh;
            const int first = mb0 + 4 * (int)blockIdx.x, last = first + 3 < mb1 ? first + 3 : mb1 - 1;
            int r_lo = first / mbw - 2, r_hi = last / mbw + 2;
            r_lo = r_lo > 0 ? r_lo : 0;
            r_hi = r_hi < mbh ? r_hi : mbh - 1;
            const uint2 *flags = (const uint2 *)(gate_done + DB_DONE_STRIDE * (blockIdx.x & (DB_DONE_COPIES - 1)));
            const int b_hi = r_hi / MI355_BAND_ROWS;
            int spins = 0, b = r_lo / MI355_BAND_ROWS;
            for (;;) {
                const uint2 f = ld64_sc1(flags + b);
                if (f.x == ref_epoch && f.y == ref_epoch) { if (++b > b_hi) break; continue; }
#ifndef PMB_POLL_SLEEP
#define PMB_POLL_SLEEP 64
#endif
                __builtin_amdgcn_s_sleep(PMB_POLL_SLEEP);
                if (++spins > DB_SPIN_MAX) { st_sc1(err, 3u); break; }
                if ((spins & 255) == 0 && ld_sc1(err)) break;
            }
            __builtin_amdgcn_fence(__ATOMIC_ACQUIRE, "agent");
        }
        __syncthreads();
        tl_last(ctx, 3);
    }
    if (mbn >= mb1) return;
    pmb_mb<ROWS, PART, T8, IR>(ctx, &LD[wave], mbn, lane, refine, pre);
    if (ROWS) {
        asm volatile("s_waitcnt vmcnt(0)" ::: "memory");
        if (lane == 0) __hip_atomic_fetch_add(row_done + (mbn / ctx->mbw) * MI355_PROG_STRIDE, 1u, __ATOMIC_RELAXED, __HIP_MEMORY_SCOPE_AGENT);
    }
    tl_last(ctx, 4);
}

__global__ __launch_bounds__(256) void copy_luma_kernel(const frame_ctx_t cv) {
    const frame_ctx_t *__restrict__ ctx = &cv;
    const int W = ctx->mbw * 16, H = ctx->mbh * 16, per_row = W / 16;
    const int i = blockIdx.x * 256 + threadIdx.x;
    if (i >= per_row * H) return;
    const int y = i / per_row, x = (i - y * per_row) * 16;
    const int sy = y < ctx->vis_h ? y : ctx->vis_h - 1;
    stg128(ctx->psrc_out + (size_t)y * ctx->stride + x, ldg128(ctx->src_y + (size_t)sy * ctx->src_stride + x));
}
void k_launch_copy_luma(const frame_ctx_t *h_ctx, hipStream_t s) {
    const int n = h_ctx->mbw * h_ctx->mbh * 16;
    hipLaunchKernelGGL(copy_luma_kernel, dim3((n + 255) / 256), dim3(256), 0, s, *h_ctx);
}

__global__ __launch_bounds__(256) void imv_to_mbi_kernel(const frame_ctx_t cv, int mb0, int mb1) {
    const frame_ctx_t *__restrict__ ctx = &cv;
    const int i = mb0 + blockIdx.x * 256 + threadIdx.x;
    if (i >= mb1) return;
    const uint2 w = ldg64(k_final_imv_dev(ctx) + i);
    const int vx = (int)(int16_t)(w.x & 0xFFFF), vy = (int)(int16_t)(w.x >> 16);
    stg32(&ctx->mbi[i].mvx, w.x);
    stg32(&ctx->mbi[i].cost, (w.y & 0xFFFFu) + (unsigned)(ctx->lambda * (mvq_bits(vx) + mvq_bits(vy))));
}

void k_launch_me(const frame_ctx_t *h_ctx, int mbw, hipStream_t s) {
    int strips = (mbw + ME_MBS - 1) / ME_MBS;
    if (h_ctx->mbh > 0) hipLaunchKernelGGL(me_kernel, dim3(strips * h_ctx->mbh), dim3(64 * ME_MBS), 0, s, *h_ctx, 0);
}
void k_launch_me_select(const frame_ctx_t *h_ctx, int mbw, const imv_t *in, imv_t *out, const imv_t *prev, int mode, hipStream_t s) {
    int n = mbw * h_ctx->mbh;
    if (n <= 0) return;
    if (mode == 2) hipLaunchKernelGGL(me_select_sparse_kernel, dim3((n + 4 * SEL_SPW - 1) / (4 * SEL_SPW)), dim3(256), 0, s, *h_ctx, 0, n, in, out, prev);
    else hipLaunchKernelGGL(me_select_kernel, dim3((n + 3) / 4), dim3(256), 0, s, *h_ctx, 0, n, in, out, prev, mode);
}
void k_launch_me_select_all(const frame_ctx_t *h_ctx, int mbw, hipStream_t s) {
    imv_t *const f[3] = {h_ctx->imv_a, h_ctx->imv_b, h_ctx->imv_c};
    for (int it = 0; it < ME_ITERS; it++) k_launch_me_select(h_ctx, mbw, f[it % 3], f[(it + 1) % 3], it ? f[(it - 1) % 3] : nullptr, it ? 2 : 1, s);
}
const imv_t *k_final_imv(const frame_ctx_t *h_ctx) { return ME_ITERS % 3 == 0 ? h_ctx->imv_a : ME_ITERS % 3 == 1 ? h_ctx->imv_b : h_ctx->imv_c; }
void k_launch_subpel(const frame_ctx_t *h_ctx, int mbw, hipStream_t s) {
    const int n = mbw * h_ctx->mbh;
    if (n > 0) hipLaunchKernelGGL(subpel_kernel, dim3((n + 3) / 4), dim3(256), 0, s, *h_ctx, 0, n);
}
typedef void (*pmb_fn_t)(const frame_ctx_t, int, int, int, const unsigned *, unsigned, unsigned *, unsigned *);
#define PMB_GATES(P, T, IR) {pmb_kernel<false, false, P, T, IR>, pmb_kernel<true, false, P, T, IR>, pmb_kernel<true, true, P, T, IR>}
static const pmb_fn_t k_pmb_table[2][4][3] = {
    {PMB_GATES(false, 0, false), PMB_GATES(true, 0, false), PMB_GATES(false, 1, false), PMB_GATES(false, 2, false)},
    {PMB_GATES(false, 0, true), {nullptr, nullptr, nullptr}, PMB_GATES(false, 1, true), PMB_GATES(false, 2, true)}};
#undef PMB_GATES
int k_launch_pmb(const frame_ctx_t *h_ctx, int mbw, const pmb_launch_t *l, hipStream_t s) {
    const int n = mbw * h_ctx->mbh;
    if (n <= 0) return 0;
    if ((l->gate != PMB_IN_ORDER && !l->gate_done) || (l->gate == PMB_GATED_ROWS && !l->row_done) || l->gate < PMB_IN_ORDER || l->gate > PMB_GATED_ROWS) return -1;
    const int ir = h_ctx->ir_c1 > 0;
    const int body = h_ctx->t8 == 2 ? 3 : h_ctx->t8 ? 2 : (!ir && h_ctx->partitions) ? 1 : 0;
    hipLaunchKernelGGL(k_pmb_table[ir][body][l->gate], dim3((n + 3) / 4), dim3(256), 0, s, *h_ctx, 0, n, l->refine, l->gate_done, l->ref_epoch, l->err, l->row_done);
    return 0;
}
```

### ceracoder_amd/csrc/mi355enc_dev.h

```cpp
#ifndef MI355ENC_DEV_H
#define MI355ENC_DEV_H
#include <stdint.h>

#ifdef __cplusplus
extern "C" {
#endif

typedef struct {
    int16_t mvx, mvy;
    uint8_t mb_type;
    uint8_t i16_mode;
    uint8_t chroma_mode;
    uint8_t qp;
    uint32_t nzmask;
    uint32_t cost;
} mb_info_t;

typedef struct {
    int16_t mvx, mvy;
    uint16_t sad;
    uint16_t bits;
} imv_t;

#define MB_LEVELS 408
#define ISAD_PER_MB 152
#define IDEC_BYTES 32
#define SURF_COLS 36
#define SURF_ROWS 35
#define SURF_U16 (SURF_ROWS * SURF_COLS)
#ifndef MI355_BAND_ROWS
#define MI355_BAND_ROWS 4
#endif
#ifndef DB_CUT_MIN_MBW
#define DB_CUT_MIN_MBW 60
#endif
#ifndef MI355_PROG_STRIDE
#define MI355_PROG_STRIDE 1024
#endif
#define IP_STRIP_BYTES 64
#define ME_ITERS 3
#define SEL_BONUS 2
#define SKIP_MARGIN_BITS 4
#define INTRA_GATE(lambda) (768u + 8u * (unsigned)(lambda))
#define DROP_MAX 12
#define DROP_SKIP 255
#define L_LUMA 0
#define L_LDC 256
#define L_CDC 272
#define L_CAC 280
#define NZ_LDC (1u << 24)
#define NZ_CBDC (1u << 25)
#define NZ_CRDC (1u << 26)
#define NZ_T8 (1u << 27)
#define PACK_BLOCKS_MAX 27

typedef struct {
    const uint8_t *src_y, *src_uv;
    const uint8_t *ref_y, *ref_uv;
    uint8_t *rec_y, *rec_uv;
    mb_info_t *mbi;
    int16_t *levels;
    uint16_t *isad;
    uint8_t *idec;
    uint8_t *dbrec;
    int32_t src_stride;
    int32_t stride;
    int32_t mbw, mbh, vis_h;
    int32_t qp, me_range, lambda;
    int32_t i4x4;
    int32_t t8;
    int32_t all_intra;
    const uint8_t *me_ref_y;
    uint8_t *psrc_out;
    uint16_t *surf;
    imv_t *imv_a, *imv_b, *imv_c;
    uint32_t epoch;
    uint32_t drop_sad;
    int32_t iac_drop;
    int32_t intra_p;
    const int8_t *qp_off;
    int32_t partitions;
    int32_t slice_rows;
    int32_t slice_dbf;
    int32_t i8;
    int32_t ir_c0, ir_c1;
    int32_t ir_clean;
} frame_ctx_t;

typedef enum { DB_ALL_INTRA, DB_P, DB_P_FOLLOWS_IP, DB_P_FUSED_IP } db_variant_t;
typedef enum { PMB_IN_ORDER, PMB_GATED, PMB_GATED_ROWS } pmb_gate_t;
typedef struct { int counted, grid; } db_wgs_t;
static inline db_wgs_t db_launch_wgs(int mbh, db_variant_t v, int parts, int qpc) {
    db_wgs_t w;
    w.counted = (parts ? 4 : 2) * ((mbh + MI355_BAND_ROWS - 1) / MI355_BAND_ROWS);
    w.grid = w.counted + (v == DB_P_FUSED_IP ? mbh : qpc ? 1 : 0);
    return w;
}
typedef struct {
    db_variant_t variant;
    int parts;
    int qpc;
    int ib_rows;
    unsigned *err;
    void *gran;
    unsigned *partab;
    unsigned *band_done;
    unsigned *started;
    const unsigned *iband_done;
    const unsigned *row_done;
    unsigned row_need;
    unsigned *ip_progress;
    uint8_t *ip_strips;
    unsigned *ip_done;
    unsigned *qpc_word; unsigned qpc_base;
    unsigned *part_cnt;
} db_launch_t;
typedef struct {
    pmb_gate_t gate;
    int refine;
    const unsigned *gate_done; unsigned ref_epoch;
    unsigned *row_done;
    unsigned *err;
} pmb_launch_t;

#ifdef __cplusplus
}
#endif

#ifdef __HIPCC__
#include <hip/hip_runtime.h>
#include "mask_host.h"
void k_launch_me(const frame_ctx_t *h_ctx, int mbw, hipStream_t s);
void k_launch_copy_luma(const frame_ctx_t *h_ctx, hipStream_t s);
void k_launch_me_select(const frame_ctx_t *h_ctx, int mbw, const imv_t *in, imv_t *out, const imv_t *prev, int mode, hipStream_t s);
void k_launch_me_select_all(const frame_ctx_t *h_ctx, int mbw, hipStream_t s);
void k_launch_intra_p(const frame_ctx_t *h_ctx, int mbw, int mbh, unsigned *d_progress , uint8_t *d_strips ,
                      unsigned *d_err, hipStream_t s);
const imv_t *k_final_imv(const frame_ctx_t *h_ctx);
void k_launch_subpel(const frame_ctx_t *h_ctx, int mbw, hipStream_t s);
int k_launch_pmb(const frame_ctx_t *h_ctx, int mbw, const pmb_launch_t *l, hipStream_t s);
void k_launch_inter(const frame_ctx_t *h_ctx, int mbw, hipStream_t s);
void k_launch_intra_analyse(const frame_ctx_t *h_ctx, int mbw, int mbh, int gate_p, hipStream_t s);
void k_launch_intra_diag(const frame_ctx_t *d_ctx, int mbw, int mbh, int diag, hipStream_t s);
void k_launch_deblock_diag(const frame_ctx_t *d_ctx, int mbw, int mbh, int diag, hipStream_t s);
int k_deblock_bands16(int mbh);
int k_launch_deblock_bands(const frame_ctx_t *h_ctx, const db_launch_t *l, hipStream_t s);
size_t k_deblock_part_bytes(int mbh);
int k_intra_band_rows(void);
size_t k_deblock_partab_bytes(int mbw, int mbh);
size_t k_deblock_gran_bytes(int mbw, int mbh);
void k_launch_wait_started(const unsigned *d_started, unsigned count, unsigned *d_err, hipStream_t s);
size_t k_deblock_done_bytes(void);
void k_launch_pad(uint8_t *y, uint8_t *uv, int stride, int vis_w, int vis_h, int W, int H, hipStream_t s);
int k_intra_diags(int mbw, int mbh);
int k_intra_bands(int mbh);
void k_launch_intra_band(const frame_ctx_t *h_ctx, int mbh, uint2 *d_gran, unsigned *d_err, unsigned *d_band_done, hipStream_t s);
void k_launch_intra_rows(const frame_ctx_t *h_ctx, int mbh, uint2 *d_gran, unsigned *d_err, unsigned *d_row_done, hipStream_t s);
int k_launch_csc(int fmt, const uint8_t *p0, const uint8_t *p1, const uint8_t *p2, int s0, int s1, int s2, uint8_t *dy, uint8_t *duv,
                 int vw, int vh, int W, int H, hipStream_t s);
int k_launch_csc2(int fmt, const uint8_t *p0, const uint8_t *p1, const uint8_t *p2, int s0, int s1, int s2, uint8_t *dy, uint8_t *duv,
                  int vw, int vh, int W, int H, const int *coef, hipStream_t s);
int k_launch_hdr(int fmt, int hlg, const uint8_t *const planes[3], const int strides[3], uint8_t *dy, uint8_t *duv, int vw, int vh, int W, int H, const int *d_tables, hipStream_t s);
int k_launch_yuv_convert(uint8_t *y, uint8_t *uv, int W, int H, const int rect[4], const int *coef, hipStream_t s);
int k_launch_adjust(uint8_t *y, uint8_t *uv, int W, int H, const int rect[4], const uint8_t *luma, const int *chroma, hipStream_t s);
int k_launch_adjust_sharpen(const uint8_t *y, uint8_t *out, int W, int H, int vw, int vh, const int rect[4], const uint8_t *luma, int amount, int thr, hipStream_t s);
int k_launch_denoise(uint8_t *y, uint8_t *uv, uint16_t *hy, uint16_t *huv, int W, int H, int vw, int vh, int lmode, int cmode, const uint8_t *tabs, hipStream_t s);
int k_launch_denoise_search(const uint8_t *y, const uint16_t *hy, unsigned *vec, int W, int H, int vw, int vh, int range, int lambda, hipStream_t s);
int k_launch_denoise_mc(uint8_t *y, uint8_t *uv, const uint16_t *hy, const uint16_t *huv, uint16_t *ny, uint16_t *nuv, const unsigned *vec, int W, int H, int vw, int vh,
                        int lmode, int cmode, const uint8_t *tabs, hipStream_t s);
#define SCALE_TABLES 5
#define SCALE_TILE_W 64
#define SCALE_TILE_H 16
#define SCALE_CHUNK 8
typedef struct {
    int in_w, in_h, out_w, out_h;
    const int *first[SCALE_TABLES];
    const int16_t *q[SCALE_TABLES];
    int taps[SCALE_TABLES];
    int hrows[3];
    int span[2];
    int geom, plain;
    int lo[SCALE_TABLES], hi[SCALE_TABLES];
    int dx, dy, dw, dh;
    int border[3];
    int cap_taps[SCALE_TABLES];
} scale_plan_t;
int k_launch_scale(int fmt, const uint8_t *p0, const uint8_t *p1, const uint8_t *p2, int s0, int s1, int s2, uint8_t *dy, uint8_t *duv,
                   int W, int H, const scale_plan_t *plan, hipStream_t s, const int *stab = nullptr);
int k_launch_warp(const uint8_t *sy, const uint8_t *suv, uint8_t *dy, uint8_t *duv, int w, int h, int W, int H, const int32_t *mesh, int kind, const uint8_t fill[3], hipStream_t s, int staging = 1);
int k_launch_stab_project(const uint8_t *luma, int stride, int step, int w, int h, unsigned *sums, hipStream_t s);
int k_launch_stab_match(const unsigned *prev, const unsigned *cur, int w, int h, int range, int leak, int prime, const int bounds[4], int *state, int *rec, hipStream_t s);
int k_launch_autolevel_measure(const uint8_t *y, const uint8_t *uv, int W, int H, const int rect[4], int vw, int vh, int full_range, int reach, unsigned *slabs, hipStream_t s);
int k_launch_autolevel_decide(const unsigned *slabs, int nslabs, unsigned NC, const int set[7], int full_range, int prime, int *state, int *rec, hipStream_t s);
int k_launch_autolevel_apply(uint8_t *y, uint8_t *uv, int W, int H, const int rect[4], int luma, int chroma, const int *rec, hipStream_t s);
int k_launch_dspatial_filter(const uint8_t *src, uint8_t *out, int W, int H, int vw, int vh, const int rect[4], int chroma, const uint8_t *weight, const int *rec, const uint8_t *tabs, hipStream_t s);
int k_launch_dspatial_measure(const uint8_t *y, int W, int H, const int rect[4], int vw, int vh, int full_range, unsigned *slabs, hipStream_t s);
int k_launch_dspatial_decide(const unsigned *slabs, int nslabs, unsigned NC, const int set[5], int prime, int *state, int *rec, hipStream_t s);
int k_launch_lut3d(uint8_t *y, uint8_t *uv, int W, int H, int vw, int vh, const int rect[4], const uint32_t *nodes, int N, int strength, const int32_t coef[19], int form, hipStream_t s);
void k_launch_pack(const mb_info_t *d_mbi, const int16_t *d_levels, int nmb, int mbw, unsigned *d_off, mb_info_t *h_mbi, int16_t *h_packed,
                   unsigned *h_hdr, const unsigned *d_err, hipStream_t s);
int k_deblock_diags(int mbw, int mbh);
void k_launch_aq(const frame_ctx_t *h_ctx, int8_t *d_off, hipStream_t s);
void k_launch_qp_chain(mb_info_t *d_mbi, int nmb, int slice_qp, int slice_mbs, hipStream_t s);
void k_launch_roi_compose(const int8_t *t, int8_t *d_off, int nmb, int have_aq, hipStream_t s);
int k_launch_mask(uint8_t *y, uint8_t *uv, int W, int H, int vw, int vh, const mask_tab_t *tab, uint8_t *res, uint8_t *pa, uint8_t *pb, size_t plane_bytes, int parts, int *launches, hipStream_t s);
#define QUALITY_WORDS 8
#define QUALITY_SHARDS 32
#define QUALITY_SHARD_STRIDE 512
#define QUALITY_TICKET_WORD 8
#define QUALITY_ACC_WORDS (QUALITY_SHARDS * QUALITY_SHARD_STRIDE)
typedef struct {
    uint8_t *y, *uv;
    int32_t stride, vw, vh, W, H;
    int32_t bx, by, bw, bh;
    int32_t gx0, gy0, gx1, gy1;
    int32_t scale, halign, shaded, nlines, maxlen;
    uint8_t text[256];
    uint8_t line_end[256];
} overlay_args_t;
void k_launch_overlay(const overlay_args_t *a, hipStream_t s);
typedef struct {
    uint8_t *y, *uv;
    const uint32_t *img;
    int32_t stride, vw, vh, W, H;
    int32_t iw, ih, x, y0, opacity;
    int32_t gx0, gy0, gx1, gy1;
} image_args_t;
int k_launch_image_prepare(uint32_t *pix, size_t n, int fmt, const int *coef, hipStream_t s);
bool k_image_grid(image_args_t *a);
void k_launch_image_blend(const image_args_t *a, hipStream_t s);
int k_launch_jpeg(const int16_t *d_coef, const uint16_t *d_qt, int hs, int vs, int comps, int vw, int vh, uint8_t *dy, uint8_t *duv, int W, int H,
                  uint8_t *d_planar, hipStream_t s);
int k_launch_orient(int method, const uint8_t *sy, int ssy, const uint8_t *suv, int ssuv, int in_w, int in_h, uint8_t *dy, uint8_t *duv, int W, int H, hipStream_t s);
int k_launch_snapshot(const uint8_t *sy, int ys, const uint8_t *suv, int uvs, int w, int h, int log2s, const void *d_tab, int16_t *levels, uint8_t *hint, hipStream_t s);
int k_launch_rate_mix(const uint8_t *a_y, const uint8_t *a_uv, const uint8_t *b_y, const uint8_t *b_uv, uint8_t *o_y, uint8_t *o_uv, uint8_t *k_y, uint8_t *k_uv,
                      int W, int H, int w256, hipStream_t s);
void k_launch_quality(const uint8_t *src_y, const uint8_t *src_uv, int src_stride, const uint8_t *rec_y, const uint8_t *rec_uv, int rec_stride,
                      int width, int height, unsigned long long *d_acc, unsigned long long *out, hipStream_t s);
#endif
#endif
```

Baseline: 7470.

## Prefetch subpel window and chroma neighborhood into LDS, batch qpel SATD reductions

Splits the reference-window and chroma loads in the P macroblock kernel into issue and consume phases so they can be issued early (optionally before integer search, controlled by a new pmb_early ctx field) and land in LDS. Chroma prediction now reads from an LDS neighborhood instead of global memory. In the non-partition path, the nine quarter-pel candidates are sampled with a table-driven operand fetch and their Hadamard sums are reduced together with batched DPP steps instead of nine separate wave reductions. It also adds LDS use per block and caps SGPRs, which may affect occupancy and register pressure.

Result: no change. 7548, median of 2 (+1.0%).

```diff
diff --git a/ceracoder_amd/csrc/enc_handle.cpp b/ceracoder_amd/csrc/enc_handle.cpp
--- a/ceracoder_amd/csrc/enc_handle.cpp
+++ b/ceracoder_amd/csrc/enc_handle.cpp
@@ -214,6 +214,11 @@
         slot_t *s = &h->slot[i];
         memset(s, 0, sizeof *s);
         HIPCHK(hipHostMalloc((void **)&s->h_ctx, sizeof(frame_ctx_t), hipHostMallocDefault));
+        memset(s->h_ctx, 0, sizeof(frame_ctx_t));
+        {
+            const char *pe = getenv("MI355ENC_PMB_EARLY");
+            s->h_ctx->pmb_early = !pe ? 0 : atoi(pe) ? 1 : 2;
+        }
         HIPCHK(hipHostMalloc((void **)&s->h_mbi, (size_t)h->nmb * sizeof(mb_info_t), hipHostMallocDefault));
         HIPCHK(hipHostMalloc((void **)&s->h_levels, (size_t)h->nmb * PACK_BLOCKS_MAX * 32, hipHostMallocDefault));
         HIPCHK(hipHostMalloc((void **)&s->h_hdr, (size_t)(4 + h->mbh) * sizeof(unsigned), hipHostMallocDefault));
diff --git a/ceracoder_amd/csrc/k_motion.hip b/ceracoder_amd/csrc/k_motion.hip
--- a/ceracoder_amd/csrc/k_motion.hip
+++ b/ceracoder_amd/csrc/k_motion.hip
@@ -296,6 +296,20 @@
 #undef SH
 #undef SJ
 }
+DEV unsigned sp_operand4(const sp_lds *L, int op, int Xs, int Ys, int l24, int l20) {
+    const int P = op & 3, dx = (op >> 2) & 1, dy = (op >> 3) & 1;
+    const unsigned long long bases = (unsigned long long)offsetof(sp_lds, G) | (unsigned long long)offsetof(sp_lds, b) << 16 | (unsigned long long)offsetof(sp_lds, h) << 32 |
+                                     (unsigned long long)offsetof(sp_lds, j) << 48;
+    const int base = (int)((bases >> (16 * P)) & 0xFFFFu), stride = (P & 1) ? SP_PS : SP_GS;
+    const int s = base + (Ys + dy + (P == 0 ? 2 : 0)) * stride + Xs + dx + ((P & 1) ? 0 : 2);
+    const unsigned *w = (const unsigned *)((const uint8_t *)L + (s & ~3) + ((P & 1) ? l20 : l24));
+    return __builtin_amdgcn_alignbyte(w[1], w[0], (unsigned)(s & 3));
+}
+DEV unsigned sp_sample4_flat(const sp_lds *L, int Xs, int Ys, int l24, int l20, int fx, int fy) {
+    const int idx = fx + 4 * fy;
+    const int code = (int)(((idx < 8 ? 0x6131212014111000ull : 0x6939292836333222ull) >> (8 * (idx & 7))) & 255u);
+    return avg4(sp_operand4(L, code & 15, Xs, Ys, l24, l20), sp_operand4(L, code >> 4, Xs, Ys, l24, l20));
+}
 DEV void sp_planes(sp_lds *L, const int lane) {
     if (lane < 54) {
         const int d = lane % 6, seg = lane / 6;
@@ -429,42 +443,111 @@
     v |= __builtin_amdgcn_update_dpp(0, v, 0x124, 0xF, 0xF, false);
     return v;
 }
+DEV void ref_word4_ask_in(const uint8_t *__restrict__ ref, int stride, int x, int y, unsigned *w) {
+    const uint8_t *b = ref + (size_t)y * stride + (x & ~3);
+    w[0] = ldg32(b); w[1] = ldg32(b + 4);
+}
+DEV unsigned ref_word4_take_in(const unsigned *w, int x) { return __builtin_amdgcn_alignbyte(w[1], w[0], (unsigned)(x & 3)); }
+DEV void ref_word4_ask_cl(const uint8_t *__restrict__ ref, int stride, int W, int H, int x, int y, unsigned *b) {
+    const uint8_t *r = ref + (size_t)clip3(0, H - 1, y) * stride;
+#pragma unroll
+    for (int i = 0; i < 4; i++) b[i] = ldg8(r + clip3(0, W - 1, x + i));
+}
+DEV unsigned ref_word4_take_cl(const unsigned *b) { return pack4((int)b[0], (int)b[1], (int)b[2], (int)b[3]); }
 DEV unsigned ref_word4(const uint8_t *__restrict__ ref, int stride, int W, int H, int x, int y, bool inside) {
-    if (inside) {
-        const uint8_t *b = ref + (size_t)y * stride + (x & ~3);
-        return __builtin_amdgcn_alignbyte(ldg32(b + 4), ldg32(b), (unsigned)(x & 3));
-    }
-    const uint8_t *r = ref + (size_t)clip3(0, H - 1, y) * stride;
-    return pack4((int)ldg8(r + clip3(0, W - 1, x)), (int)ldg8(r + clip3(0, W - 1, x + 1)), (int)ldg8(r + clip3(0, W - 1, x + 2)), (int)ldg8(r + clip3(0, W - 1, x + 3)));
-}
-DEV void chroma_pred4(const frame_ctx_t *__restrict__ ctx, int lane, int x0, int y0, int W, int H, int mvx, int mvy, int *pd) {
+    unsigned w[2], b[4];
+    if (inside) { ref_word4_ask_in(ref, stride, x, y, w); return ref_word4_take_in(w, x); }
+    ref_word4_ask_cl(ref, stride, W, H, x, y, b);
+    return ref_word4_take_cl(b);
+}
+DEV int chroma_pred4_room(int x0, int y0, int W, int H, int mvx, int mvy) {
+    const int x = (x0 >> 1) + (mvx >> 3), y = (y0 >> 1) + (mvy >> 3);
+    return x | ((W >> 1) - 9 - x) | y | ((H >> 1) - 9 - y);
+}
+DEV bool chroma_pred4_inside(int x0, int y0, int W, int H, int mvx, int mvy) { return chroma_pred4_room(x0, y0, W, H, mvx, mvy) >= 0; }
+DEV void chroma_pred4_ask_in(const frame_ctx_t *__restrict__ ctx, int lane, int x0, int y0, int mvx, int mvy, unsigned *w) {
+    const int stride = ctx->stride;
+    const int py = (lane >> 2) & 3, cby = (lane >> 4) & 1, c = (lane >> 1) & 1, cbx = lane & 1;
+    const int o = 2 * ((x0 >> 1) + cbx * 4 + (mvx >> 3)) + c;
+    const uint8_t *r0 = ctx->ref_uv + (size_t)((y0 >> 1) + cby * 4 + py + (mvy >> 3)) * stride + (o & ~3), *r1 = r0 + stride;
+    w[0] = ldg32(r0); w[1] = ldg32(r0 + 4); w[2] = ldg32(r0 + 8); w[3] = ldg32(r1); w[4] = ldg32(r1 + 4); w[5] = ldg32(r1 + 8);
+}
+DEV void chroma_pred4_ask_cl(const frame_ctx_t *__restrict__ ctx, int lane, int x0, int y0, int W, int H, int mvx, int mvy, unsigned *b) {
     const int stride = ctx->stride;
     const int py = (lane >> 2) & 3, cby = (lane >> 4) & 1, c = (lane >> 1) & 1, cbx = lane & 1;
     const int cx0 = x0 >> 1, cy0 = y0 >> 1, cw = W >> 1, ch = H >> 1;
     const int cy = cby * 4 + py, cxb = cbx * 4;
-    const int xi = mvx >> 3, yi = mvy >> 3, xf = mvx & 7, yf = mvy & 7;
+    const int xi = mvx >> 3, yi = mvy >> 3;
     const uint8_t *__restrict__ rf = ctx->ref_uv;
+    const int ya = clip3(0, ch - 1, cy0 + cy + yi), yb = clip3(0, ch - 1, cy0 + cy + yi + 1);
+#pragma unroll
+    for (int i = 0; i < 5; i++) {
+        const int xx = clip3(0, cw - 1, cx0 + cxb + i + xi);
+        b[i] = ldg8(rf + (size_t)ya * stride + 2 * xx + c);
+        b[5 + i] = ldg8(rf + (size_t)yb * stride + 2 * xx + c);
+    }
+}
+DEV void chroma_bilin4(const int *A, const int *B, int mvx, int mvy, int *pd) {
+    const int xf = mvx & 7, yf = mvy & 7;
+    const int w00 = (8 - xf) * (8 - yf), w10 = xf * (8 - yf), w01 = (8 - xf) * yf, w11 = xf * yf;
+#pragma unroll
+    for (int i = 0; i < 4; i++) pd[i] = (w00 * A[i] + w10 * A[i + 1] + w01 * B[i] + w11 * B[i + 1] + 32) >> 6;
+}
+DEV void chroma_bilin4_words(unsigned a0, unsigned a1, unsigned a2, unsigned b0, unsigned b1, unsigned b2, int a, int mvx, int mvy, int *pd) {
+    const unsigned sa0 = __builtin_amdgcn_alignbyte(a1, a0, (unsigned)a), sa1 = __builtin_amdgcn_alignbyte(a2, a1, (unsigned)a);
+    const unsigned sb0 = __builtin_amdgcn_alignbyte(b1, b0, (unsigned)a), sb1 = __builtin_amdgcn_alignbyte(b2, b1, (unsigned)a);
+    const int A[5] = {byte_of(sa0, 0), byte_of(sa0, 2), byte_of(sa1, 0), byte_of(sa1, 2), (int)((a2 >> (8 * a)) & 255)};
+    const int B[5] = {byte_of(sb0, 0), byte_of(sb0, 2), byte_of(sb1, 0), byte_of(sb1, 2), (int)((b2 >> (8 * a)) & 255)};
+    chroma_bilin4(A, B, mvx, mvy, pd);
+}
+DEV void chroma_pred4_take_in(int lane, int x0, int mvx, int mvy, const unsigned *w, int *pd) {
+    const int c = (lane >> 1) & 1, cbx = lane & 1;
+    chroma_bilin4_words(w[0], w[1], w[2], w[3], w[4], w[5], (2 * ((x0 >> 1) + cbx * 4 + (mvx >> 3)) + c) & 3, mvx, mvy, pd);
+}
+DEV void chroma_pred4_take_cl(int mvx, int mvy, const unsigned *b, int *pd) {
     int A[5], B[5];
-    if (cx0 + xi >= 0 && cx0 + xi + 9 <= cw && cy0 + yi >= 0 && cy0 + yi + 9 <= ch) {
-        const int o = 2 * (cx0 + cxb + xi) + c, a = o & 3;
-        const uint8_t *r0 = rf + (size_t)(cy0 + cy + yi) * stride + (o & ~3), *r1 = r0 + stride;
-        const unsigned a0 = ldg32(r0), a1 = ldg32(r0 + 4), a2 = ldg32(r0 + 8), b0 = ldg32(r1), b1 = ldg32(r1 + 4), b2 = ldg32(r1 + 8);
-        const unsigned sa0 = __builtin_amdgcn_alignbyte(a1, a0, (unsigned)a), sa1 = __builtin_amdgcn_alignbyte(a2, a1, (unsigned)a);
-        const unsigned sb0 = __builtin_amdgcn_alignbyte(b1, b0, (unsigned)a), sb1 = __builtin_amdgcn_alignbyte(b2, b1, (unsigned)a);
-        A[0] = byte_of(sa0, 0); A[1] = byte_of(sa0, 2); A[2] = byte_of(sa1, 0); A[3] = byte_of(sa1, 2); A[4] = (int)((a2 >> (8 * a)) & 255);
-        B[0] = byte_of(sb0, 0); B[1] = byte_of(sb0, 2); B[2] = byte_of(sb1, 0); B[3] = byte_of(sb1, 2); B[4] = (int)((b2 >> (8 * a)) & 255);
-    } else {
-        const int ya = clip3(0, ch - 1, cy0 + cy + yi), yb = clip3(0, ch - 1, cy0 + cy + yi + 1);
-#pragma unroll
-        for (int i = 0; i < 5; i++) {
-            const int xx = clip3(0, cw - 1, cx0 + cxb + i + xi);
-            A[i] = (int)ldg8(rf + (size_t)ya * stride + 2 * xx + c);
-            B[i] = (int)ldg8(rf + (size_t)yb * stride + 2 * xx + c);
-        }
-    }
-    const int w00 = (8 - xf) * (8 - yf), w10 = xf * (8 - yf), w01 = (8 - xf) * yf, w11 = xf * yf;
-#pragma unroll
-    for (int i = 0; i < 4; i++) pd[i] = (w00 * A[i] + w10 * A[i + 1] + w01 * B[i] + w11 * B[i + 1] + 32) >> 6;
+#pragma unroll
+    for (int i = 0; i < 5; i++) { A[i] = (int)b[i]; B[i] = (int)b[5 + i]; }
+    chroma_bilin4(A, B, mvx, mvy, pd);
+}
+DEV void chroma_pred4(const frame_ctx_t *__restrict__ ctx, int lane, int x0, int y0, int W, int H, int mvx, int mvy, int *pd) {
+    unsigned w[6], b[10];
+    if (chroma_pred4_inside(x0, y0, W, H, mvx, mvy)) { chroma_pred4_ask_in(ctx, lane, x0, y0, mvx, mvy, w); chroma_pred4_take_in(lane, x0, mvx, mvy, w, pd); }
+    else { chroma_pred4_ask_cl(ctx, lane, x0, y0, W, H, mvx, mvy, b); chroma_pred4_take_cl(mvx, mvy, b, pd); }
+}
+#define CN_STRIDE 24
+#define CN_BYTES (10 * CN_STRIDE)
+DEV int chroma_nb_room(int nx, int ny, int W, int H) { return nx | ny | (W - CN_STRIDE - ((2 * nx) & ~3)) | ((H >> 1) - 10 - ny); }
+DEV bool chroma_nb_inside(int nx, int ny, int W, int H) { return chroma_nb_room(nx, ny, W, H) >= 0; }
+DEV unsigned chroma_nb_ask_in(const frame_ctx_t *__restrict__ ctx, int lane, int nx, int ny) {
+    const int i = lane < 60 ? lane : 59, r = i / 6, d = i - r * 6;
+    return ldg32(ctx->ref_uv + (size_t)(ny + r) * ctx->stride + ((2 * nx) & ~3) + 4 * d);
+}
+DEV void chroma_nb_take_in(uint8_t *CN, int lane, unsigned w) { if (lane < 60) *(unsigned *)&CN[4 * lane] = w; }
+DEV void chroma_nb_ask_cl(const frame_ctx_t *__restrict__ ctx, int lane, int nx, int ny, int W, int H, unsigned *b) {
+    const int cw = W >> 1, ch = H >> 1;
+#pragma unroll
+    for (int k = 0; k < 4; k++) {
+        int i = lane + 64 * k;
+        i = i < 200 ? i : 199;
+        const int r = i / 20, o = i - r * 20;
+        b[k] = ldg8(ctx->ref_uv + (size_t)clip3(0, ch - 1, ny + r) * ctx->stride + 2 * clip3(0, cw - 1, nx + (o >> 1)) + (o & 1));
+    }
+}
+DEV void chroma_nb_take_cl(uint8_t *CN, int lane, const unsigned *b) {
+#pragma unroll
+    for (int k = 0; k < 4; k++) {
+        const int i = lane + 64 * k, r = i / 20, o = i - r * 20;
+        if (i < 200) CN[r * CN_STRIDE + o] = (uint8_t)b[k];
+    }
+}
+DEV void chroma_pred4_lds(const uint8_t *CN, int a0, int xi0, int yi0, int lane, int mvx, int mvy, int *pd) {
+    const int py = (lane >> 2) & 3, cby = (lane >> 4) & 1, c = (lane >> 1) & 1, cbx = lane & 1;
+    const int cy = cby * 4 + py, cxb = cbx * 4;
+    const int dx = (mvx >> 3) - xi0, dy = (mvy >> 3) - yi0;
+    const int o = a0 + 2 * (cxb + dx) + c;
+    const unsigned *r0 = (const unsigned *)(CN + (cy + dy) * CN_STRIDE + (o & ~3)), *r1 = r0 + CN_STRIDE / 4;
+    chroma_bilin4_words(r0[0], r0[1], r0[2], r1[0], r1[1], r1[2], o & 3, mvx, mvy, pd);
 }
 DEV unsigned pmb_luma_tq(const dev_tables *T, int lane, unsigned curw, unsigned pw, int qp, bool decimate, int *lev, int *x) {
     const int py = (lane >> 2) & 3, fy = ((py & 1) << 1) | (py >> 1);
@@ -499,7 +582,9 @@
     const int rb = lane & 15, rbx = blkx(rb) >> 2, rby = blky(rb) >> 2;
     return (unsigned)(__ballot(lane < 16 && ((t >> (16 * rby + rbx)) & 1)) & 0xFFFFull);
 }
-DEV unsigned pmb_satd(int lane, unsigned curw, unsigned pw) {
+DEV int pmb_had(int lane, unsigned curw, unsigned pw);
+DEV unsigned pmb_satd(int lane, unsigned curw, unsigned pw) { return (unsigned)wave64_sum(pmb_had(lane, curw, pw)); }
+DEV int pmb_had(int lane, unsigned curw, unsigned pw) {
     const int py = (lane >> 2) & 3, s1 = py < 2 ? 1 : -1, s2 = (py & 1) ? -1 : 1;
     const int d0 = byte_of(curw, 0) - byte_of(pw, 0), d1 = byte_of(curw, 1) - byte_of(pw, 1), d2 = byte_of(curw, 2) - byte_of(pw, 2), d3 = byte_of(curw, 3) - byte_of(pw, 3);
     const int a = d0 + d3, b = d1 + d2, c = d1 - d2, e = d0 - d3;
@@ -511,7 +596,22 @@
         const int w = mad24(u, s2, row_xor4(u));
         acc += iabs(w);
     }
-    return (unsigned)wave64_sum(acc);
+    return acc;
+}
+template <int N>
+DEV void wave64_sum_lane63(int *v) {
+#pragma unroll
+    for (int i = 0; i < N; i++) v[i] += __builtin_amdgcn_update_dpp(0, v[i], 0x128, 0xF, 0xF, false);
+#pragma unroll
+    for (int i = 0; i < N; i++) v[i] += __builtin_amdgcn_update_dpp(0, v[i], 0x124, 0xF, 0xF, false);
+#pragma unroll
+    for (int i = 0; i < N; i++) v[i] += __builtin_amdgcn_update_dpp(0, v[i], 0x4E, 0xF, 0xF, false);
+#pragma unroll
+    for (int i = 0; i < N; i++) v[i] += __builtin_amdgcn_update_dpp(0, v[i], 0xB1, 0xF, 0xF, false);
+#pragma unroll
+    for (int i = 0; i < N; i++) v[i] += __builtin_amdgcn_update_dpp(0, v[i], 0x142, 0xA, 0xF, false);
+#pragma unroll
+    for (int i = 0; i < N; i++) v[i] += __builtin_amdgcn_update_dpp(0, v[i], 0x143, 0xC, 0xF, false);
 }
 DEV unsigned pmb_sa8d(int lane, unsigned curw, unsigned pw) {
     const int s0 = (lane & 1) ? -1 : 1, s1 = (lane & 4) ? -1 : 1, s2 = (lane & 8) ? -1 : 1, s3 = (lane & 16) ? -1 : 1;
@@ -661,13 +761,15 @@
 }
 DEV unsigned part_total(unsigned g) { g += (unsigned)quad_xor<2>((int)g); return g + (unsigned)__shfl_xor((int)g, 32, 64); }
 #ifdef PMB_PROF
-#define PMB_NPH 11
+#define PMB_NPH 14
 #define PMB_MARK(k) do { const unsigned long long t1_ = __builtin_readcyclecounter(); ph_[k] = t1_ - t0_; t0_ = t1_; } while (0)
-#define PMB_MARK0() unsigned long long ph_[PMB_NPH] = {0, 0, 0, 0, 0, 0, 0, 0, 0, 0, 0}; unsigned long long t0_ = __builtin_readcyclecounter()
+#define PMB_MARK0() unsigned long long ph_[PMB_NPH] = {0, 0, 0, 0, 0, 0, 0, 0, 0, 0, 0, 0, 0, 0}; unsigned long long t0_ = __builtin_readcyclecounter()
+#define PMB_NOTE_AHEAD(e) (ph_[13] = (e) ? 2 : 1)
 #define PMB_FLUSH() do { if (lane == 0) for (int k_ = 0; k_ < PMB_NPH; k_++) stg32((unsigned *)ctx->dbrec + (size_t)mbn * 16 + k_, (unsigned)ph_[k_]); } while (0)
 #else
 #define PMB_MARK(k) ((void)0)
 #define PMB_MARK0() ((void)0)
+#define PMB_NOTE_AHEAD(e) ((void)0)
 #define PMB_FLUSH() ((void)0)
 #endif
 struct pmb_pre_t { uint2 selfw; fpred_t fp; unsigned curw; uint2 sw; unsigned ds; uint4 dw; };
@@ -710,11 +812,52 @@
         st_mbinfo_x<SC1>(mb, m);
     }
 }
+DEV int sp_window_room(int ix, int iy, int W, int H) { return (ix - 3) | (iy - 3) | (W - 28 - ((ix - 3) & ~3)) | (H - 20 - iy); }
+DEV bool sp_window_inside(int ix, int iy, int W, int H) { return sp_window_room(ix, iy, W, H) >= 0; }
+DEV void sp_window_ask_in(const uint8_t *__restrict__ ref, int stride, int ix, int iy, int lane, unsigned *w) {
+    const uint8_t *base = ref + (size_t)(iy - 3) * stride + ((ix - 3) & ~3);
+#pragma unroll
+    for (int k = 0; k < 3; k++) {
+        int i = lane + 64 * k;
+        i = i < 23 * 6 ? i : 23 * 6 - 1;
+        const int r = i / 6, d = i - r * 6;
+        w[2 * k] = ldg32(base + (size_t)r * stride + 4 * d); w[2 * k + 1] = ldg32(base + (size_t)r * stride + 4 * d + 4);
+    }
+}
+DEV void sp_window_take_in(sp_lds *L, int ix, int lane, const unsigned *w) {
+    const int a = (ix - 3) & 3;
+#pragma unroll
+    for (int k = 0; k < 3; k++) {
+        const int i = lane + 64 * k, r = i / 6, d = i - r * 6;
+        if (i < 23 * 6) *(unsigned *)&L->G[r * SP_GS + 4 * d] = __builtin_amdgcn_alignbyte(w[2 * k + 1], w[2 * k], (unsigned)a);
+    }
+}
+DEV void sp_window_ask_cl(const uint8_t *__restrict__ ref, int stride, int W, int H, int ix, int iy, int lane, unsigned *b) {
+#pragma unroll
+    for (int k = 0; k < 9; k++) {
+        int i = lane + 64 * k;
+        i = i < 23 * 23 ? i : 23 * 23 - 1;
+        const int r = i / 23, c = i - r * 23;
+        b[k] = ldg8(ref + (size_t)clip3(0, H - 1, iy - 3 + r) * stride + clip3(0, W - 1, ix - 3 + c));
+    }
+}
+DEV void sp_window_take_cl(sp_lds *L, int lane, const unsigned *b) {
+#pragma unroll
+    for (int k = 0; k < 9; k++) {
+        const int i = lane + 64 * k, r = i / 23, c = i - r * 23;
+        if (i < 23 * 23) L->G[r * SP_GS + c] = (uint8_t)b[k];
+    }
+}
+#ifndef PMB_EARLY_BITS
+#define PMB_EARLY_BITS 64
+#endif
+DEV bool pmb_expects_refinement(bool pass, unsigned ds, int lambda) { return !pass && ds > (unsigned)(lambda * PMB_EARLY_BITS); }
 template <bool SC1, bool PART, int T8, bool IR>
-DEV void pmb_mb(const frame_ctx_t *__restrict__ ctx, sp_lds *L, const int mbn, const int lane, const int refine, const pmb_pre_t &pre) {
+DEV void pmb_mb(const frame_ctx_t *__restrict__ ctx, sp_lds *L, uint8_t *CN, const int mbn, const int lane, const int refine, const pmb_pre_t &pre) {
     const int mbw = ctx->mbw, mbh = ctx->mbh, stride = ctx->stride, W = mbw * 16, H = mbh * 16, qp = mb_qp_dev(ctx, mbn), lambda = ctx->lambda;
     const int my = mbn / mbw, mx = mbn - my * mbw, x0 = mx * 16, y0 = my * 16;
     const dev_tables *T = &g_tab;
+    constexpr bool AHEAD = !IR;
     PMB_MARK0();
     const uint2 selfw = pre.selfw;
     int imx = (int)(int16_t)(selfw.x & 0xFFFF);
@@ -738,18 +881,38 @@
         PMB_FLUSH();
         return;
     }
+    if (IR && !ir_ok(ctx, mx, imx)) imx = ir_max_whole(ctx, mx);
+    const uint8_t *__restrict__ ref = ctx->ref_y;
+    unsigned ww[6], nw = 0;
+    int ahead;
     {
         const unsigned ds = pre.ds;
         const bool skip_ok = !IR || ir_ok(ctx, mx, fp.sx);
         bool pass = ctx->drop_sad && ds < ctx->drop_sad && skip_ok;
         const bool worth = ds <= di + (unsigned)(lambda * SKIP_MARGIN_BITS) && skip_ok;
+        const int X = x0 + (fp.sx >> 2), Y = y0 + (fp.sy >> 2);
+        const int sroom = X | Y | (W - 16 - X) | (H - 16 - Y);
+        const bool inside = sroom >= 0;
+        const int ix = x0 + (imx >> 2), iy = y0 + (imy >> 2), nx = (x0 >> 1) + ((imx - 3) >> 3), ny = (y0 >> 1) + ((imy - 3) >> 3);
+        const int room = sroom | chroma_pred4_room(x0, y0, W, H, fp.sx, fp.sy) | sp_window_room(ix, iy, W, H) | chroma_nb_room(nx, ny, W, H);
+        ahead = __builtin_amdgcn_readfirstlane((int)(AHEAD && (pass || worth) && room >= 0 && (ctx->pmb_early == 1 || (ctx->pmb_early == 0 && pmb_expects_refinement(pass, ds, lambda)))));
+        PMB_NOTE_AHEAD(ahead);
         PMB_MARK(0);
         if (pass || worth) {
-            const int X = x0 + (fp.sx >> 2), Y = y0 + (fp.sy >> 2);
-            const bool inside = X >= 0 && Y >= 0 && X + 16 <= W && Y + 16 <= H;
-            const unsigned pw = ref_word4(ctx->ref_y, stride, W, H, X + pc, Y + pr, inside);
+            unsigned pw;
             int pd[4];
-            chroma_pred4(ctx, lane, x0, y0, W, H, fp.sx, fp.sy, pd);
+            if (ahead) {
+                unsigned sw[2], cw[6];
+                ref_word4_ask_in(ref, stride, X + pc, Y + pr, sw);
+                chroma_pred4_ask_in(ctx, lane, x0, y0, fp.sx, fp.sy, cw);
+                sp_window_ask_in(ref, stride, ix, iy, lane, ww);
+                nw = chroma_nb_ask_in(ctx, lane, nx, ny);
+                pw = ref_word4_take_in(sw, X + pc);
+                chroma_pred4_take_in(lane, x0, fp.sx, fp.sy, cw, pd);
+            } else {
+                pw = ref_word4(ref, stride, W, H, X + pc, Y + pr, inside);
+                chroma_pred4(ctx, lane, x0, y0, W, H, fp.sx, fp.sy, pd);
+            }
             if (!pass) {
                 int lev[4], x[4];
                 if (pmb_luma_tq(T, lane, curw, pw, qp, true, lev, x) == 0) {
@@ -771,25 +934,29 @@
             }
         }
     }
-    if (IR && !ir_ok(ctx, mx, imx)) imx = ir_max_whole(ctx, mx);
+    asm volatile("" : "+s"(imx));
     const int ix = x0 + (imx >> 2), iy = y0 + (imy >> 2);
-    const uint8_t *__restrict__ ref = ctx->ref_y;
-    if (ix - 3 >= 0 && iy - 3 >= 0 && ((ix - 3) & ~3) + 28 <= W && iy + 19 < H) {
-        const int a = (ix - 3) & 3;
-        const uint8_t *base = ref + (size_t)(iy - 3) * stride + ((ix - 3) & ~3);
-        for (int i = lane; i < 23 * 6; i += 64) {
-            const int r = i / 6, d = i - r * 6;
-            const unsigned w0 = ldg32(base + (size_t)r * stride + 4 * d), w1 = ldg32(base + (size_t)r * stride + 4 * d + 4);
-            *(unsigned *)&L->G[r * SP_GS + 4 * d] = __builtin_amdgcn_alignbyte(w1, w0, (unsigned)a);
-        }
-    } else
-        for (int i = lane; i < 23 * 23; i += 64) {
-            int r = i / 23, c = i - r * 23;
-            int yy = clip3(0, H - 1, iy - 3 + r), xx = clip3(0, W - 1, ix - 3 + c);
-            L->G[r * SP_GS + c] = (uint8_t)ldg8(ref + (size_t)yy * stride + xx);
-        }
+    const int xi0 = (imx - 3) >> 3, yi0 = (imy - 3) >> 3, nx = (x0 >> 1) + xi0, ny = (y0 >> 1) + yi0;
+    const bool win_in = sp_window_inside(ix, iy, W, H), cn_in = chroma_nb_inside(nx, ny, W, H);
+    if (ahead) {
+        asm volatile("s_waitcnt vmcnt(0)" ::: "memory");
+        PMB_MARK(2);
+        int ln = lane;
+        asm volatile("" : "+v"(ln));
+        sp_window_take_in(L, ix, ln, ww);
+        chroma_nb_take_in(CN, ln, nw);
+    } else {
+        unsigned wb[9], nb[4];
+        if (win_in) sp_window_ask_in(ref, stride, ix, iy, lane, ww); else sp_window_ask_cl(ref, stride, W, H, ix, iy, lane, wb);
+        if (cn_in) nw = chroma_nb_ask_in(ctx, lane, nx, ny); else chroma_nb_ask_cl(ctx, lane, nx, ny, W, H, nb);
+        asm volatile("s_waitcnt vmcnt(0)" ::: "memory");
+        PMB_MARK(2);
+        if (win_in) sp_window_take_in(L, ix, lane, ww); else sp_window_take_cl(L, lane, wb);
+        if (cn_in) chroma_nb_take_in(CN, lane, nw); else chroma_nb_take_cl(CN, lane, nb);
+    }
+    const int cn_a = cn_in ? (2 * nx) & 3 : 0;
     WAVE_SYNC();
-    PMB_MARK(2);
+    PMB_MARK(3);
     int bqx = imx, bqy = imy;
     unsigned q0 = 0, qh[4] = {0, 0, 0, 0}, qq[4] = {0, 0, 0, 0};
     int hbx = imx, hby = imy;
@@ -800,10 +967,10 @@
     } else
         best = (unsigned)wave64_sum((int)__builtin_amdgcn_sad_u8(curw, sp_sample4(L, 1 + pc, 1 + pr, 0, 0), 0u)) +
                (unsigned)(lambda * (mvq_bits(imx - fp.px) + mvq_bits(imy - fp.py)));
-    PMB_MARK(3);
+    PMB_MARK(4);
     if (refine) {
         sp_planes(L, lane);
-        PMB_MARK(4);
+        PMB_MARK(5);
         {
             const int cqx = bqx, cqy = bqy;
             unsigned acc[4] = {0, 0, 0, 0};
@@ -830,8 +997,8 @@
             }
         }
         hbx = bqx; hby = bqy;
-        PMB_MARK(5);
-        {
+        PMB_MARK(6);
+        if constexpr (PART) {
             const int cqx = bqx, cqy = bqy;
             {
                 const int ox = cqx - imx, oy = cqy - imy;
@@ -844,18 +1011,45 @@
                 const int qx = cqx + (k % 3 - 1), qy = cqy + (k / 3 - 1);
                 const int ox = qx - imx, oy = qy - imy;
                 const unsigned cw = sp_sample4(L, 1 + (ox >> 2) + pc, 1 + (oy >> 2) + pr, ox & 3, oy & 3);
-                if (PART) {
-                    const int c8 = k < 4 ? k : k - 1;
-                    const unsigned g = part_gsum(__builtin_amdgcn_sad_u8(curw, cw, 0u)) << (16 * (c8 & 1));
-                    qq[0] |= (c8 >> 1) == 0 ? g : 0u; qq[1] |= (c8 >> 1) == 1 ? g : 0u; qq[2] |= (c8 >> 1) == 2 ? g : 0u; qq[3] |= (c8 >> 1) == 3 ? g : 0u;
-                }
+                const int c8 = k < 4 ? k : k - 1;
+                const unsigned g = part_gsum(__builtin_amdgcn_sad_u8(curw, cw, 0u)) << (16 * (c8 & 1));
+                qq[0] |= (c8 >> 1) == 0 ? g : 0u; qq[1] |= (c8 >> 1) == 1 ? g : 0u; qq[2] |= (c8 >> 1) == 2 ? g : 0u; qq[3] |= (c8 >> 1) == 3 ? g : 0u;
                 const unsigned d = pmb_satd(lane, curw, cw) >> 1;
                 const unsigned cost = d + (unsigned)(lambda * (mvq_bits(qx - fp.px) + mvq_bits(qy - fp.py)));
-                if (cost < best && (!IR || ir_ok(ctx, mx, qx))) { best = cost; bqx = qx; bqy = qy; }
-            }
-        }
-    }
-    PMB_MARK(6);
+                if (cost < best) { best = cost; bqx = qx; bqy = qy; }
+            }
+            PMB_MARK(7);
+        } else {
+            const int cqx = bqx, cqy = bqy;
+            int hs[9];
+            unsigned cw[9];
+            const int l24 = pr * SP_GS + pc, l20 = pr * SP_PS + pc;
+#pragma unroll
+            for (int c = 0; c < 9; c++) {
+                const int k = c == 0 ? 4 : c < 5 ? c - 1 : c;
+                const int qx = cqx + (k % 3 - 1), qy = cqy + (k / 3 - 1);
+                const int ox = qx - imx, oy = qy - imy;
+                cw[c] = sp_sample4_flat(L, 1 + (ox >> 2), 1 + (oy >> 2), l24, l20, ox & 3, oy & 3);
+            }
+#pragma unroll
+            for (int c = 0; c < 9; c++) hs[c] = pmb_had(lane, curw, cw[c]);
+            wave64_sum_lane63<9>(hs);
+            PMB_MARK(7);
+            unsigned key = 0xFFFFFFFFu;
+#pragma unroll
+            for (int c = 0; c < 9; c++) {
+                const int k = c == 0 ? 4 : c < 5 ? c - 1 : c;
+                const int qx = cqx + (k % 3 - 1), qy = cqy + (k / 3 - 1);
+                const unsigned cost = ((unsigned)hs[c] >> 1) + (unsigned)(lambda * (mvq_bits(qx - fp.px) + mvq_bits(qy - fp.py)));
+                const unsigned kc = (c == 0 || !IR || ir_ok(ctx, mx, qx)) ? (cost << 4) | (unsigned)c : 0xFFFFFFFFu;
+                key = kc < key ? kc : key;
+            }
+            key = (unsigned)__builtin_amdgcn_readlane((int)key, 63);
+            const int c = (int)(key & 15u), k = c == 0 ? 4 : c < 5 ? c - 1 : c;
+            best = key >> 4; bqx = cqx + (k % 3 - 1); bqy = cqy + (k / 3 - 1);
+        }
+    }
+    PMB_MARK(8);
     const int ox = bqx - imx, oy = bqy - imy;
     unsigned pw = sp_sample4(L, 1 + (ox >> 2) + pc, 1 + (oy >> 2) + pr, ox & 3, oy & 3);
     unsigned dsad = (unsigned)wave64_sum((int)__builtin_amdgcn_sad_u8(curw, pw, 0u));
@@ -907,18 +1101,18 @@
             return;
         }
     }
-    PMB_MARK(7);
+    PMB_MARK(9);
     int pd[4];
     unsigned slot = 0;
     if (PART && shape) {
         const int src = (((lane >> 4) & 1) << 5) | ((lane & 1) << 1);
         const int cvx = __shfl(lvx, src, 64), cvy = __shfl(lvy, src, 64);
-        chroma_pred4(ctx, lane, x0, y0, W, H, cvx, cvy, pd);
+        chroma_pred4_lds(CN, cn_a, xi0, yi0, lane, cvx, cvy, pd);
         const unsigned mine = ((unsigned)(uint16_t)lvx) | ((unsigned)(uint16_t)lvy << 16);
         const unsigned v1 = (unsigned)__shfl((int)mine, shape == 1 ? 32 : 2, 64), v2 = (unsigned)__shfl((int)mine, 32, 64), v3 = (unsigned)__shfl((int)mine, 34, 64);
         slot = lane == 0 ? v1 : (shape == 3 && lane == 1) ? v2 : (shape == 3 && lane == 2) ? v3 : 0u;
         bqx = __builtin_amdgcn_readfirstlane(lvx); bqy = __builtin_amdgcn_readfirstlane(lvy);
-    } else chroma_pred4(ctx, lane, x0, y0, W, H, bqx, bqy, pd);
+    } else chroma_pred4_lds(CN, cn_a, xi0, yi0, lane, bqx, bqy, pd);
     if (ctx->drop_sad && dsad < ctx->drop_sad) {
         pmb_store_pred_only<SC1>(ctx, lv, lane, x0, y0, pw, pd);
         if (PART && shape && lane < 8) stx32<SC1>(lv + L_LDC + 2 * lane, slot);
@@ -930,7 +1124,7 @@
         PMB_FLUSH();
         return;
     }
-    PMB_MARK(8);
+    PMB_MARK(10);
     unsigned nz_luma;
     const bool t8 = T8 == 1 || (T8 == 2 && pmb_pick_t8(lane, curw, pw));
     if (t8) {
@@ -950,10 +1144,10 @@
         for (int i = 0; i < 4; i++) o[i] = clip255(byte_of(pw, i) + ((inv_col(x[i], cb) + 32) >> 6));
         stx32<SC1>(ctx->rec_y + (size_t)(y0 + pr) * stride + x0 + pc, pack4(o[0], o[1], o[2], o[3]));
     }
-    PMB_MARK(9);
+    PMB_MARK(11);
     unsigned nz_c = 0, dc_c = 0;
     chroma_rows4(ctx, T, lv, x0 >> 1, y0 >> 1, lane, pd, sv, qp, false, true, nullptr, nz_c, dc_c, true, 0, SC1);
-    PMB_MARK(10);
+    PMB_MARK(12);
     if (lane == 0) {
         unsigned nzm = nz_luma | (nz_c << 16);
         if (dc_c & 1) nzm |= NZ_CBDC;
@@ -969,9 +1163,10 @@
 }
 
 template <bool GATED, bool ROWS, bool PART, int T8, bool IR = false>
-__global__ __launch_bounds__(256) void pmb_kernel(const frame_ctx_t cv, int mb0, int mb1, int refine, const unsigned *__restrict__ gate_done, unsigned ref_epoch, unsigned *err, unsigned *row_done) {
+__global__ __launch_bounds__(256) __attribute__((amdgpu_num_sgpr(82))) void pmb_kernel(const frame_ctx_t cv, int mb0, int mb1, int refine, const unsigned *__restrict__ gate_done, unsigned ref_epoch, unsigned *err, unsigned *row_done) {
     const frame_ctx_t *__restrict__ ctx = &cv;
     __shared__ __attribute__((aligned(16))) sp_lds LD[4];
+    __shared__ __attribute__((aligned(16))) uint8_t CN[4][CN_BYTES];
     const int lane = threadIdx.x & 63, wave = __builtin_amdgcn_readfirstlane(threadIdx.x >> 6);
     const int mbn = mb0 + 4 * (int)blockIdx.x + wave;
     if (mb0 == 0 && blockIdx.x == 0) tl_first(ctx, 2);
@@ -1003,7 +1198,7 @@
         tl_last(ctx, 3);
     }
     if (mbn >= mb1) return;
-    pmb_mb<ROWS, PART, T8, IR>(ctx, &LD[wave], mbn, lane, refine, pre);
+    pmb_mb<ROWS, PART, T8, IR>(ctx, &LD[wave], CN[wave], mbn, lane, refine, pre);
     if (ROWS) {
         asm volatile("s_waitcnt vmcnt(0)" ::: "memory");
         if (lane == 0) __hip_atomic_fetch_add(row_done + (mbn / ctx->mbw) * MI355_PROG_STRIDE, 1u, __ATOMIC_RELAXED, __HIP_MEMORY_SCOPE_AGENT);
diff --git a/ceracoder_amd/csrc/mi355enc_dev.h b/ceracoder_amd/csrc/mi355enc_dev.h
--- a/ceracoder_amd/csrc/mi355enc_dev.h
+++ b/ceracoder_amd/csrc/mi355enc_dev.h
@@ -85,6 +85,7 @@
     int32_t i8;
     int32_t ir_c0, ir_c1;
     int32_t ir_clean;
+    int32_t pmb_early;
 } frame_ctx_t;
 
 typedef enum { DB_ALL_INTRA, DB_P, DB_P_FOLLOWS_IP, DB_P_FUSED_IP } db_variant_t;
```
